# s-elkazdadi/ddp-pinocchio

Measured on AMD Instinct MI355X. Metric: DDP iterations/sec (fwd+bwd sweep), Talos nq=38 T=200, higher is better.
Workload: dtype f64

## Files before the change

ddp_pinocchio_amd/csrc/internal.h:

```cpp
#pragma once

#include <hip/hip_runtime.h>
#include <stdint.h>

#include <vector>

#include "bwd_jobs.h"
#include "cost_block.h"
#include "ddp_hip/ddp_hip.h"

#define DDP_MAXJ DDP_HIP_MAX_JOINTS

struct DevModel {
  int32_t kind, nv;
  int32_t ff, nj, nq, pad0_;
  double mass, length;
  double gravity[3];
  double dt, c;
  int32_t parent[DDP_MAXJ];
  int32_t jtype[DDP_MAXJ];
  double axis[DDP_MAXJ][3];
  double Rp[DDP_MAXJ][9];
  double pp[DDP_MAXJ][3];
  double I6[DDP_MAXJ][21];
  int32_t has_child[DDP_MAXJ];
  int32_t first_contrib[DDP_MAXJ];
  int32_t last_child[DDP_MAXJ];
  int32_t slot_up[DDP_MAXJ];
  int32_t slot_down[DDP_MAXJ];
  int32_t n_slots;
  int32_t n_levels, max_level_width;
  int32_t lvl_start[DDP_MAXJ + 1];
  int32_t lvl_joint[DDP_MAXJ];
  int32_t child_start[DDP_MAXJ + 1];
  int32_t child_list[DDP_MAXJ];
  int32_t eq_kind, eq_advance, frame_joint, first_order_fd, fd_mode, pad_;
  double frame_off[3];
};

struct Dims {
  int64_t T, n, m, nx, nv, batch;
  int64_t Etot;
  int64_t emax;
};

struct SeqBuf {
  double* ptr = nullptr;
  int64_t size = 0;
};

struct DevSwitches {
  bool generic_bwd = false;
  bool k3_no_sym = false;
  bool k3_no_half = false;
  bool k3_no_pack = false;
  bool k3h_column_jobs = false;
  bool fxx_full = false;
  bool no_static = false;
  bool no_qcache = false;
  bool qcache_dense = false;
  bool cfg_full_aba = false;
  bool ana_own_aba = false;
  bool ana_split = false;
  bool ana_eq_kernel = false;
  bool bwd_no_graph = false;
  bool solve_sync = false;
  bool fwd_no_pipe = false;
  bool lin_serial = false;
  int32_t lin_forks = 0;
  int32_t bwd_cbx = 0, bwd_cbu = 0;
  int64_t qws_bt = 0;
  int64_t ana_bt = 0;
};

struct SweepPlan {
  bool fast;
  bool sym_ok;
  bool sym;
  int32_t half_mode;
  bool packed;
};

enum class LinFirst : int32_t {
  Base,
  AnalyticSmall,
  AnalyticWave,
  AnalyticFF,
  FdStatic,
  FdGeneric,
};
enum class LinSecond : int32_t {
  None,
  Zeros,
  Mode2Static,
  Mode2Caches,
  Mode2Plain,
  Mode1Small,
  Mode1Wave,
};
enum class LinEq : int32_t {
  None,
  PerLane,
  Analytic,
  Chain,
};
enum LinFork : uint32_t {
  LIN_FORK_CFG = 1,
  LIN_FORK_SPINE = 2,
  LIN_FORK_DEFAULT = LIN_FORK_CFG | LIN_FORK_SPINE,
};
enum class LinEqJac : int32_t { None, Fd, FfLookahead };
enum class LinEqSecond : int32_t { None, Zeros, Mode2, Mode1Small, Mode1Wave };
struct LinPlan {
  int32_t refuse = 0;
  int32_t nj = 0;
  int32_t topo = 0;
  LinFirst first = LinFirst::Base;
  LinSecond second = LinSecond::None;
  LinEq eq = LinEq::None;
  LinEqJac eq_jac = LinEqJac::None;
  LinEqSecond eq_second = LinEqSecond::None;
  bool eq_inline = false;
  bool accel_static = false;
  bool accel_with_u = false;
  bool m1_fused = false;
  int32_t ncfg = 0, nvcfg = 0;
  bool qc_sparse = false;
  bool has_tensors = false;
  bool skip_top = false;
  bool skip_qv_mirror = false;
  bool pack = false;
  bool ws_lin = false, ws_qws = false, ws_qws2 = false;
  bool ws_ana_T = false, ws_ana_M = false, ws_ana_M0 = false, ws_ana_A = false, ws_ana_F = false;
  bool ws_eq = false;
  bool ana_sliced = false;
  int64_t eq_fxk_off = 0, eq_c_off = 0, eq_words = 0;
  uint32_t forks = 0;
  int32_t lin_path = 0, first_order = 0;
};
DevSwitches read_switches();
LinPlan lin_plan_decide(const DevModel& m, const Dims& d, uint32_t flags, const DevSwitches& sw, int topo_id, bool sweep_sym_ok);

enum class TensorOrigin : int32_t {
  Unknown,
  Symmetric,
  Stencil,
  Analytic1,
};
struct TensorState {
  TensorOrigin origin = TensorOrigin::Unknown;
  bool mirror_pending = false;
  bool packed = false;
};

struct LinCall {
  bool ana_A_fresh = false;
  bool ana_M0_fresh = false;
  bool fuu_zero = false;
};

struct ProfSlot {
  std::vector<hipEvent_t> starts, stops;
  size_t used = 0;
  double total_ms = 0;
  int64_t launches = 0;
};

struct ddp_hip_ctx {
  int device = 0;
  int cu_count = 0;
  uint32_t flags = 0;
  hipStream_t stream = nullptr;
  Dims d{};
  std::vector<int64_t> ne_h, Epre_h;
  int64_t* ne_d = nullptr;
  int64_t* Epre_d = nullptr;
  double* target_d = nullptr;
  DevModel model_h{};
  DevModel* model_d = nullptr;
  SeqBuf seq[DDP_HIP_SEQ_COUNT];
  DevSwitches sw;

  double* ws_V = nullptr;
  double* ws_Q = nullptr;
  double* reg_d = nullptr;
  double* mu_d = nullptr;
  int32_t* status_d = nullptr;
  int64_t* restarts_d = nullptr;
  BwdJob* jobs_d = nullptr;
  BwdJob* jobs_half_d = nullptr;
  int32_t njobs_half = 0;
  K3hUnit* units_half_d = nullptr;
  int32_t njobs_units = 0;
  TensorState tensors;
  BwdJob* jobs_sym_d = nullptr;
  int32_t njobs = 0;
  int32_t cbx = 0, cbu = 0;
  struct BwdGraph { const void* key_x = nullptr; uint64_t key_misc = 0; hipGraphExec_t exec = nullptr; hipGraph_t graph = nullptr; };
  BwdGraph bwd_graph[4];
  int bwd_graph_next = 0;

  double* fw_x = nullptr;
  double* fw_u = nullptr;
  double* fw_dcost = nullptr;
  double* fw_cost = nullptr;
  double* fw_cost_old = nullptr;
  double* step_d = nullptr;
  int32_t* fw_state_d = nullptr;
  double* fw_dcost_acc_d = nullptr;
  int32_t n_alpha_max = 8;
  double* pick_pair_d = nullptr;

  double* eq_ws = nullptr;
  double* lin_ws = nullptr;
  LinPlan plan;
  double* lin_qws = nullptr;
  int64_t lin_qws_bt = 0;
  double* lin_qws2 = nullptr;
  hipStream_t lin_stream2 = nullptr;
  hipEvent_t lin_ev_up[2] = {nullptr, nullptr}, lin_ev_dn[2] = {nullptr, nullptr};
  hipEvent_t lin_ev_fork = nullptr, lin_ev_done = nullptr, lin_ev_rows = nullptr;
  bool lin_side_busy = false;
  double* ana_T = nullptr;
  double* ana_M = nullptr;
  double* ana_F = nullptr;
  double* ana_M0 = nullptr;
  double* ana_A = nullptr;
  int64_t ana_nbt = 0;

  std::vector<int32_t> active_h;
  bool all_active = true;

  CostBlock cost[COST_COUNT];
  int32_t fc_nf = 0;
  int32_t fc_joint[DDP_HIP_MAX_COST_FRAMES] = {};
  double fc_off[DDP_HIP_MAX_COST_FRAMES][3] = {};
  int32_t ob_np = 0, ob_no = 0;
  int32_t ob_joint[DDP_HIP_MAX_COLLISION_POINTS] = {};
  double ob_off[DDP_HIP_MAX_COLLISION_POINTS][3] = {};
  double ob_radius[DDP_HIP_MAX_COLLISION_POINTS] = {};
  int32_t ob_kind[DDP_HIP_MAX_OBSTACLES] = {};
  double* ob_clear_d = nullptr;
  int32_t sc_np = 0, sc_npair = 0;
  int32_t sc_joint[DDP_HIP_MAX_COLLISION_POINTS] = {};
  double sc_off[DDP_HIP_MAX_COLLISION_POINTS][3] = {};
  double sc_radius[DDP_HIP_MAX_COLLISION_POINTS] = {};
  int32_t sc_pa[DDP_HIP_MAX_COLLISION_PAIRS] = {}, sc_pb[DDP_HIP_MAX_COLLISION_PAIRS] = {};
  double* sc_clear_d = nullptr;
  int32_t cp_nc = 0, cp_npair = 0;
  int32_t cp_joint[DDP_HIP_MAX_CAPSULES] = {};
  double cp_end[DDP_HIP_MAX_CAPSULES][2][3] = {};
  double cp_radius[DDP_HIP_MAX_CAPSULES] = {};
  int32_t cp_pa[DDP_HIP_MAX_CAPSULE_PAIRS] = {}, cp_kind[DDP_HIP_MAX_CAPSULE_PAIRS] = {}, cp_pb[DDP_HIP_MAX_CAPSULE_PAIRS] = {};
  double* cp_clear_d = nullptr;
  int32_t rf_np = 0;
  int32_t rf_ja[DDP_HIP_MAX_FRAME_PAIRS] = {}, rf_jb[DDP_HIP_MAX_FRAME_PAIRS] = {};
  double rf_offa[DDP_HIP_MAX_FRAME_PAIRS][3] = {}, rf_offb[DDP_HIP_MAX_FRAME_PAIRS][3] = {};
  double* rf_err_d = nullptr;
  int32_t fa_nf = 0;
  int32_t fa_joint[DDP_HIP_MAX_AIM_FRAMES] = {};
  double fa_off[DDP_HIP_MAX_AIM_FRAMES][3] = {}, fa_axis[DDP_HIP_MAX_AIM_FRAMES][3] = {};
  double* fa_err_d = nullptr;

  int32_t br_np = 0;
  double* ja_acc_d = nullptr;
  double* br_margin_d = nullptr;

  bool box_dirty = false;

  void* adv_tab_d = nullptr;
  double* adv_x0_d = nullptr;
  int32_t adv_narr = 0;
  int64_t adv_blocks = 0;
  bool adv_dirty = true;
  std::vector<double> adv_mu_h, adv_step_h;

  bool async_mode = false;
  uint32_t profile_mask = 0;
  ProfSlot prof[DDP_HIP_K_COUNT];
};

#define HIP_TRY(expr)                                   \
  do {                                                  \
    hipError_t e__ = (expr);                            \
    if (e__ != hipSuccess) { (void)hipGetLastError(); return DDP_HIP_E_HIP; } \
  } while (0)

#define END_SYNC(ctx) do { if (!(ctx)->async_mode) HIP_TRY(hipStreamSynchronize((ctx)->stream)); } while (0)

inline hipError_t lin_fork(ddp_hip_ctx* ctx) {
  hipError_t e = hipEventRecord(ctx->lin_ev_fork, ctx->stream);
  if (e == hipSuccess) e = hipStreamWaitEvent(ctx->lin_stream2, ctx->lin_ev_fork, 0);
  if (e == hipSuccess) ctx->lin_side_busy = true;
  return e;
}
inline hipError_t lin_join(ddp_hip_ctx* ctx) {
  if (!ctx->lin_side_busy) return hipSuccess;
  hipError_t e = hipEventRecord(ctx->lin_ev_done, ctx->lin_stream2);
  if (e == hipSuccess) e = hipStreamWaitEvent(ctx->stream, ctx->lin_ev_done, 0);
  if (e != hipSuccess) { (void)hipGetLastError(); (void)hipStreamSynchronize(ctx->lin_stream2); }
  ctx->lin_side_busy = false;
  return e;
}
struct LinJoin {
  ddp_hip_ctx* ctx;
  explicit LinJoin(ddp_hip_ctx* c) : ctx(c) {}
  LinJoin(const LinJoin&) = delete;
  LinJoin& operator=(const LinJoin&) = delete;
  ~LinJoin() { (void)lin_join(ctx); }
};

void prof_begin(ddp_hip_ctx* ctx, int kid, hipStream_t stream = nullptr);
void prof_end(ddp_hip_ctx* ctx, int kid, hipStream_t stream = nullptr);

int bwd_setup(ddp_hip_ctx* ctx);
SweepPlan sweep_plan(const ddp_hip_ctx* ctx);
void bwd_teardown(ddp_hip_ctx* ctx);
int bwd_lds_check(const ddp_hip_ctx* ctx);
int box_check(ddp_hip_ctx* ctx);
int fwd_setup(ddp_hip_ctx* ctx);
bool fwd_lat_supported(const ddp_hip_ctx* ctx);
void fwd_teardown(ddp_hip_ctx* ctx);
void adv_teardown(ddp_hip_ctx* ctx);
int lin_setup(ddp_hip_ctx* ctx);
int tensors_written_outside(ddp_hip_ctx* ctx, int seq);
int lin_materialize_fxx(ddp_hip_ctx* ctx);
void lin_teardown(ddp_hip_ctx* ctx);

int pick_local_launch(ddp_hip_ctx* ctx, int64_t rank, int64_t nranks, double* out_pair, hipStream_t stream);
int pick_final_launch(const double* pairs, int G, double* out_pair, hipStream_t stream);

static inline int64_t seq_block_offset_regular(int64_t t, int64_t stride) { return t * stride; }
```

ddp_pinocchio_amd/csrc/lin.hip:

```cpp
#include <float.h>
#include <math.h>
#include <stdlib.h>

#include "balance_region_cost.h"
#include "capsule_cost.h"
#include "com_cost.h"
#include "control_grav_cost.h"
#include "frame_aim_cost.h"
#include "frame_cost.h"
#include "frame_vel_cost.h"
#include "internal.h"
#include "joint_accel_cost.h"
#include "lin_common.h"
#include "momentum_cost.h"
#include "obstacle_cost.h"
#include "rbd.h"
#include "rbd_deriv.h"
#include "relative_frame_cost.h"
#include "self_collision_cost.h"
#include "state_limits.h"

namespace {


// ... 1101 lines not shown
    else { for (int i = m.nq; i < nx; ++i) xb[i] = xa[i]; rbd::eval_f_q<NJ>(m, xa, xb); }
    for (int i = 0; i < nx; ++i) { xa[i] = xb[i]; p.eq_xk[(gid * K + k) * nx + i] = xb[i]; }
  }
  double* C = p.eq_c + gid * (int64_t)p.d.emax * n;
  for (int i = 0; i < e * n; ++i) C[i] = 0.0;
  const double* target = p.target + Eo;
  if (m.eq_kind == DDP_HIP_EQ_CONFIG) {
    for (int i = 0; i < e; ++i) { p.eq_val[Eb + i] = xa[i] - target[i]; C[i + i * e] = 1.0; }
  } else {
    double pos[3], J[3 * NJ];
    rbd::frame_position<NJ>(m, xa, pos, J);
    for (int i = 0; i < e; ++i) p.eq_val[Eb + i] = pos[i] - target[i];
    for (int j = 0; j < nv; ++j)
      for (int i = 0; i < e; ++i) C[i + j * e] = J[i + 3 * j];
  }
}

template <int NJ>
__global__ void eq_fdjac_kernel(LinParams p) {
  const int64_t gid = (int64_t)blockIdx.x * blockDim.x + threadIdx.x;
  const int64_t T = p.d.T;
  const DevModel& m = *p.model;
  const int n = 2 * m.nv, K = m.eq_advance;
  if (K < 2 || gid >= p.d.batch * T * (K - 1) * n) return;
  const int j = (int)(gid % n);
  const int k = (int)((gid / n) % (K - 1));
  const int64_t bt = gid / ((int64_t)n * (K - 1));
  const int b = (int)(bt / T);
  const int64_t t = bt % T;
  if (p.ne[t] == 0) return;
  double x[2 * NJ + 1], u[NJ], f[2 * NJ + 1];
  const int nx = (int)p.d.nx;
  const double* xk = p.eq_xk + (bt * K + k) * nx;
  const double* xk1 = p.eq_xk + (bt * K + k + 1) * nx;
  const double* us = p.u + ((int64_t)b * T + t) * m.nv;
  for (int i = 0; i < nx; ++i) x[i] = xk[i];
  for (int i = 0; i < m.nv; ++i) u[i] = us[i];
  const double eps = sqrt(DBL_EPSILON);
  lie::perturb_x(m, x, j, eps);
  double* col = p.eq_fxk + (bt * (K - 1) + k) * (int64_t)n * n + (int64_t)j * n;
  if (k == K - 2 && !m.ff) {
    const int nv = m.nv;
    for (int i = 0; i < nv; ++i) { const double vo = m.dt * x[nv + i]; const double fq = x[i] + vo; col[i] = (fq - xk1[i]) / eps; }
    for (int i = nv; i < n; ++i) col[i] = 0.0;
    return;
  }
  rbd::eval_f<NJ>(m, x, u, f);
  if (m.ff) {
    double df[2 * NJ];
    lie::difference_x(m, xk1, f, df);
    for (int i = 0; i < n; ++i) col[i] = df[i] / eps;
  } else {
    for (int i = 0; i < n; ++i) col[i] = (f[i] - xk1[i]) / eps;
  }
}

__global__ void eq_combine_kernel(LinParams p) {
  const int64_t bt = blockIdx.x;
  const int64_t T = p.d.T;
  const int b = (int)(bt / T);
  const int64_t t = bt % T;
  const int e = (int)p.ne[t];
  if (e == 0) return;
  const int n = (int)p.d.n, mm = (int)p.d.m, K = p.model->eq_advance;
  const int64_t Eb = (int64_t)b * p.d.Etot + p.Epre[t];
  extern __shared__ double sm[];
  double* ex = sm;
  double* tmp = sm + (int64_t)p.d.emax * n;
  const double* C = p.eq_c + bt * (int64_t)p.d.emax * n;
  for (int i = threadIdx.x; i < e * n; i += blockDim.x) ex[i] = C[i];
  __syncthreads();
  for (int k = K - 2; k >= 0; --k) {
    const double* F = p.eq_fxk + (bt * (K - 1) + k) * (int64_t)n * n;
    for (int idx = threadIdx.x; idx < e * n; idx += blockDim.x) {
      const int i = idx % e, j = idx / e;
      double s = 0;
      for (int l = 0; l < n; ++l) s += ex[i + l * e] * F[l + (int64_t)j * n];
      tmp[idx] = s;
    }
    __syncthreads();
    for (int i = threadIdx.x; i < e * n; i += blockDim.x) ex[i] = tmp[i];
    __syncthreads();
  }
  const double* fx = p.fx + bt * n * n;
  const double* fu = p.fu + bt * n * mm;
  for (int idx = threadIdx.x; idx < e * n; idx += blockDim.x) {
    const int i = idx % e, j = idx / e;
    double s = 0;
    for (int l = 0; l < n; ++l) s += ex[i + l * e] * fx[l + j * n];
    p.eq_x[Eb * n + idx] = s;
  }
  for (int idx = threadIdx.x; idx < e * mm; idx += blockDim.x) {
    const int i = idx % e, j = idx / e;
    double s = 0;
    for (int l = 0; l < n; ++l) s += ex[i + l * e] * fu[l + j * n];
    p.eq_u[Eb * mm + idx] = s;
  }
}

#define MAXADV 4

template <int NJ>
__global__ void eq_first_kernel(LinParams p) {
  const int64_t gid = (int64_t)blockIdx.x * blockDim.x + threadIdx.x;
  const int64_t T = p.d.T;
  if (gid >= p.d.batch * T) return;
  const int b = (int)(gid / T);
  const int64_t t = gid % T;
  const int e = (int)p.ne[t];
  if (e == 0) return;
  const DevModel& m = *p.model;
  const int n = (int)p.d.n, mm = (int)p.d.m;
  const int64_t Eo = p.Epre[t], Eb = (int64_t)b * p.d.Etot + Eo;
  double x[2 * NJ], u[NJ];
  load_xu<NJ>(p, b, t, x, u);
  eq_first_order<NJ, MAXADV>(m, p.target + Eo, e, x, u, p.eq_x + Eb * n, p.eq_u + Eb * mm, p.eq_val + Eb);
}

template <int NJ>
__global__ void second_m1_kernel(LinParams p, int is_eq) {
  const int64_t gid = (int64_t)blockIdx.x * blockDim.x + threadIdx.x;
  const int64_t T = p.d.T;
  const int n = (int)p.d.n, mm = (int)p.d.m;
  const int W = n + mm;
  if (gid >= p.d.batch * T * W) return;
  const int i = (int)(gid % W);
  const int64_t bt = gid / W;
  const int b = (int)(bt / T);
  const int64_t t = bt % T;
  const DevModel& m = *p.model;
  constexpr int N = 2 * NJ, M = NJ, EM = NJ > 3 ? NJ : 3;
  double x[N], u[M];
  load_xu<NJ>(p, b, t, x, u);
  const double eps = sqrt(DBL_EPSILON);
  const bool at_x = i < n;
  const int idx = at_x ? i : i - n;
  if (at_x) x[idx] = x[idx] + eps; else u[idx] = u[idx] + eps;
  if (!is_eq) {
    double fx_[N * N], fu_[N * M], out_[N];
    first_order_f<NJ>(m, x, u, fx_, fu_, out_);
    const double* ox = p.fx + bt * n * n;
    const double* ou = p.fu + bt * n * mm;
    const int o = n;
    if (at_x) {
      for (int k = 0; k < o; ++k) {
        for (int j = 0; j < n; ++j) p.fxx[bt * n * n * n + k + (int64_t)j * o + (int64_t)idx * o * n] = (fx_[k + j * o] - ox[k + j * o]) / eps;
        for (int j = 0; j < mm; ++j) p.fux[bt * n * mm * n + k + (int64_t)j * o + (int64_t)idx * o * mm] = (fu_[k + j * o] - ou[k + j * o]) / eps;
      }
    } else {
      for (int k = 0; k < o; ++k)
        for (int j = 0; j < mm; ++j) p.fuu[bt * n * mm * mm + k + (int64_t)j * o + (int64_t)idx * o * mm] = (fu_[k + j * o] - ou[k + j * o]) / eps;
    }
  } else {
    const int e = (int)p.ne[t];
    if (e == 0) return;
    const int64_t Eo = p.Epre[t], Eb = (int64_t)b * p.d.Etot + Eo;
    double ex_[EM * N], eu_[EM * M], out_[EM];
    eq_first_order<NJ, MAXADV>(m, p.target + Eo, e, x, u, ex_, eu_, out_);
    const double* ox = p.eq_x + Eb * n;
    const double* ou = p.eq_u + Eb * mm;
    const int o = e;
    if (at_x) {
      for (int k = 0; k < o; ++k) {
        for (int j = 0; j < n; ++j) p.eq_xx[Eb * n * n + k + (int64_t)j * o + (int64_t)idx * o * n] = (ex_[k + j * o] - ox[k + j * o]) / eps;
        for (int j = 0; j < mm; ++j) p.eq_ux[Eb * mm * n + k + (int64_t)j * o + (int64_t)idx * o * mm] = (eu_[k + j * o] - ou[k + j * o]) / eps;
      }
    } else {
      for (int k = 0; k < o; ++k)
        for (int j = 0; j < mm; ++j) p.eq_uu[Eb * mm * mm + k + (int64_t)j * o + (int64_t)idx * o * mm] = (eu_[k + j * o] - ou[k + j * o]) / eps;
    }
  }
}

template <int NJ>
__global__ void eq_second_m2_kernel(LinParams p, int stage) {
  const int64_t gid = (int64_t)blockIdx.x * blockDim.x + threadIdx.x;
  const int64_t T = p.d.T;
  const int n = (int)p.d.n, mm = (int)p.d.m;
  const int W = n + mm;
  const int64_t P = stage == 0 ? W : (int64_t)W * (W - 1) / 2;
  if (gid >= p.d.batch * T * P) return;
  const int64_t pid = gid % P;
  const int64_t bt = gid / P;
  const int b = (int)(bt / T);
  const int64_t t = bt % T;
  const int e = (int)p.ne[t];
  if (e == 0) return;
  int i, j;
  if (stage == 0) { i = (int)pid; j = -1; }
  else {
    i = (int)floor(((2.0 * W - 1.0) - sqrt((2.0 * W - 1.0) * (2.0 * W - 1.0) - 8.0 * (double)pid)) * 0.5);
    if (i < 0) i = 0;
    while ((int64_t)i * (2 * W - i - 1) / 2 > pid) --i;
    while ((int64_t)(i + 1) * (2 * W - i - 2) / 2 <= pid) ++i;
    j = (int)(pid - (int64_t)i * (2 * W - i - 1) / 2) + i + 1;
  }
  const DevModel& m = *p.model;
  constexpr int EM = NJ > 3 ? NJ : 3;
  double x[2 * NJ + 1], u[NJ], f1[EM];
  load_xu<NJ>(p, b, t, x, u);
  const double eps = sqrt(sqrt(DBL_EPSILON));
  const double eps2 = eps * eps;
  const int64_t Eo = p.Epre[t], Eb = (int64_t)b * p.d.Etot + Eo;
  const double* f0 = p.eq_val + Eb;
  double* exx = p.eq_xx + Eb * n * n;
  double* eux = p.eq_ux + Eb * mm * n;
  double* euu = p.eq_uu + Eb * mm * mm;
  const bool at_x_1 = i < n;
  const int idx_1 = at_x_1 ? i : i - n;
  const bool both_base = stage != 0 && m.ff && i < 6 && j < 6;
  if (both_base) {
    double nu[6] = {0, 0, 0, 0, 0, 0}, q7[7];
    nu[i] = eps; nu[j] = eps;
    lie::se3_integrate(x, nu, q7);
    for (int k = 0; k < 7; ++k) x[k] = q7[k];
  } else if (at_x_1) lie::perturb_x(m, x, idx_1, eps); else u[idx_1] = u[idx_1] + eps;
  const double* fcol_1 = at_x_1 ? p.eq_x + Eb * n + (int64_t)idx_1 * e : p.eq_u + Eb * mm + (int64_t)idx_1 * e;
  const int L1 = at_x_1 ? n : mm;
  double* tensor_1 = at_x_1 ? exx : euu;
  if (stage == 0) {
    eq_eval<NJ>(m, p.target + Eo, e, x, u, f1);
    for (int k = 0; k < e; ++k) {
      double df = f1[k] - f0[k];
      df -= eps * fcol_1[k];
      df *= 2;
      tensor_1[k + (int64_t)idx_1 * e + (int64_t)idx_1 * e * L1] = df / eps2;
    }
    return;
  }
  const bool at_x_2 = j < n;
  const int idx_2 = at_x_2 ? j : j - n;
  if (both_base) {} else if (at_x_2) lie::perturb_x(m, x, idx_2, eps); else u[idx_2] = u[idx_2] + eps;
  const double* fcol_2 = at_x_2 ? p.eq_x + Eb * n + (int64_t)idx_2 * e : p.eq_u + Eb * mm + (int64_t)idx_2 * e;
  const int L2 = at_x_2 ? n : mm;
  const double* tensor_2 = at_x_2 ? exx : euu;
  double* tensor;
  int L;
  if (at_x_1) { if (at_x_2) { tensor = exx; L = n; } else { tensor = eux; L = mm; } }
  else { tensor = euu; L = mm; }
  eq_eval<NJ>(m, p.target + Eo, e, x, u, f1);
  for (int k = 0; k < e; ++k) {
    double df = f1[k] - f0[k];
    df -= eps * fcol_1[k];
    df -= eps * fcol_2[k];
    df *= 2;
    const double val = 0.5 * (df / eps2 - tensor_1[k + (int64_t)idx_1 * e + (int64_t)idx_1 * e * L1] -
                              tensor_2[k + (int64_t)idx_2 * e + (int64_t)idx_2 * e * L2]);
    tensor[k + (int64_t)idx_2 * e + (int64_t)idx_1 * e * L] = val;
    if (at_x_1 == at_x_2) tensor[k + (int64_t)idx_1 * e + (int64_t)idx_2 * e * L] = val;
  }
}

__global__ void tensor_mirror_kernel(double* Tn, int64_t BT, int n, int L) {
  const int64_t per = (int64_t)n * L * L, total = BT * per;
  for (int64_t g = (int64_t)blockIdx.x * blockDim.x + threadIdx.x; g < total; g += (int64_t)gridDim.x * blockDim.x) {
    const int64_t bt = g / per, r = g % per;
    const int k = (int)(r % n), j = (int)((r / n) % L), c = (int)(r / ((int64_t)n * L));
    if (j >= c) continue;
    double* T = Tn + bt * per;
    T[k + (int64_t)j * n + (int64_t)c * n * L] = T[k + (int64_t)c * n + (int64_t)j * n * L];
  }
}

__global__ void tensor_zero_top_kernel(double* Tn, int64_t total_cols, int n, int nv) {
  const int64_t total = total_cols * nv;
  for (int64_t g = (int64_t)blockIdx.x * blockDim.x + threadIdx.x; g < total; g += (int64_t)gridDim.x * blockDim.x) {
    const int64_t col = g / nv;
    Tn[col * n + (g % nv)] = 0.0;
  }
}

constexpr int UNPACK_BS = 256;
__global__ __launch_bounds__(UNPACK_BS) void tensor_unpack_kernel(double* fxx, double* fux, double* fuu, int n, int m, int nv) {
  extern __shared__ __attribute__((aligned(16))) double s_rec[];
  const int per = 2 * n + m;
  const int64_t bt = blockIdx.x / per;
  const int s = (int)(blockIdx.x % per);
  double* slab;
  int L, c;
  bool tops;
  if (s < n) { c = s; L = n; tops = true; slab = fxx + (bt * n + c) * (int64_t)n * n; }
  else if (s < 2 * n) { c = s - n; L = m; tops = true; slab = fux + (bt * n + c) * (int64_t)n * m; }
  else { c = s - 2 * n; L = m; tops = false; slab = fuu + (bt * m + c) * (int64_t)n * m; }
  const int R = nv + 2, words = L * R;
  for (int e = threadIdx.x; e < words; e += UNPACK_BS) s_rec[e] = slab[e];
  __syncthreads();
  const int r0 = c % nv;
  for (int e = threadIdx.x; e < L * n; e += UNPACK_BS) {
    const int j = e / n, k = e - j * n;
    const double* rec = s_rec + j * R;
    double v = 0.0;
    if (k >= nv) v = rec[2 + (k - nv)];
    else if (tops && k == r0) v = rec[0];
    else if (tops && L == n && k == j % nv) v = rec[1];
    slab[e] = v;
  }
}

int64_t lin_qc_per_bt(const ddp_hip_ctx* ctx) {
  const LinPlan& pl = ctx->plan;
  return pl.qc_sparse ? lin_static_qc_per_bt(pl.topo) : (int64_t)pl.ncfg * ctx->d.nv * rbd::QC_STRIDE;
}

LinParams make_params(ddp_hip_ctx* ctx) {
  LinParams p{};
  p.d = ctx->d;
  p.model = ctx->model_d;
  p.ne = ctx->ne_d;
  p.Epre = ctx->Epre_d;
  p.target = ctx->target_d;
  auto S = [&](int s) { return ctx->seq[s].ptr; };
  p.x = S(DDP_HIP_SEQ_X); p.u = S(DDP_HIP_SEQ_U);
  p.lfx = S(DDP_HIP_SEQ_LFX); p.lfxx = S(DDP_HIP_SEQ_LFXX);
  p.lx = S(DDP_HIP_SEQ_LX); p.lu = S(DDP_HIP_SEQ_LU); p.lxx = S(DDP_HIP_SEQ_LXX); p.lux = S(DDP_HIP_SEQ_LUX); p.luu = S(DDP_HIP_SEQ_LUU);
  p.f_val = S(DDP_HIP_SEQ_F_VAL); p.fx = S(DDP_HIP_SEQ_FX); p.fu = S(DDP_HIP_SEQ_FU);
  p.fxx = S(DDP_HIP_SEQ_FXX); p.fux = S(DDP_HIP_SEQ_FUX); p.fuu = S(DDP_HIP_SEQ_FUU);
  p.eq_val = S(DDP_HIP_SEQ_EQ_VAL); p.eq_x = S(DDP_HIP_SEQ_EQ_X); p.eq_u = S(DDP_HIP_SEQ_EQ_U);
  p.eq_xx = S(DDP_HIP_SEQ_EQ_XX); p.eq_ux = S(DDP_HIP_SEQ_EQ_UX); p.eq_uu = S(DDP_HIP_SEQ_EQ_UU);
  const LinPlan& pl = ctx->plan;
  p.has_tensors = pl.has_tensors ? 1 : 0;
  p.skip_top = pl.skip_top ? 1 : 0;
  p.skip_qv_mirror = pl.skip_qv_mirror ? 1 : 0;
  p.pack = pl.pack ? 1 : 0;
  p.eq_xk = ctx->eq_ws;
  if (p.eq_xk) { p.eq_fxk = p.eq_xk + pl.eq_fxk_off; p.eq_c = p.eq_xk + pl.eq_c_off; }
  p.qcache = ctx->lin_ws;
  p.ncfg = pl.ncfg; p.nvcfg = pl.nvcfg;
  p.qc_sparse = pl.qc_sparse ? 1 : 0;
  p.qc_bt = lin_qc_per_bt(ctx);
  p.vcache = p.qcache ? p.qcache + ctx->d.batch * ctx->d.T * p.qc_bt : nullptr;
  p.xref = S(DDP_HIP_SEQ_COST_XREF); p.wx = S(DDP_HIP_SEQ_COST_WX); p.uref = S(DDP_HIP_SEQ_COST_UREF); p.wu = S(DDP_HIP_SEQ_COST_WU);
  return p;
}

inline unsigned blocks_for(int64_t total) { return (unsigned)((total + LBS - 1) / LBS); }

template <int NJ>
int eq_second_order(ddp_hip_ctx* ctx, const LinParams& p, LinCall& call, uint32_t stages) {
  const Dims& d = ctx->d;
  const int64_t BT = d.batch * d.T;
  const int W = (int)(d.n + d.m);
  const int64_t P = (int64_t)W * (W - 1) / 2;
  switch (ctx->plan.eq_second) {
    case LinEqSecond::None: break;
    case LinEqSecond::Mode2:
      hipLaunchKernelGGL((eq_second_m2_kernel<NJ>), dim3(blocks_for(BT * W)), dim3(LBS), 0, ctx->stream, p, 0);
      hipLaunchKernelGGL((eq_second_m2_kernel<NJ>), dim3(blocks_for(BT * P)), dim3(LBS), 0, ctx->stream, p, 1);
      break;
    case LinEqSecond::Mode1Small:
      if constexpr (NJ <= 6) hipLaunchKernelGGL((second_m1_kernel<NJ>), dim3(blocks_for(BT * W)), dim3(LBS), 0, ctx->stream, p, 1);
      break;
    case LinEqSecond::Mode1Wave: {
      const int fl = LIN_ANA_EQ | ((stages & DDP_HIP_LIN_SECOND) ? LIN_ANA_F : 0);
      if (fl & LIN_ANA_F) prof_begin(ctx, DDP_HIP_K_LIN_SECOND);
      const int rc_ = lin_analytic_launch(ctx, p, call, 1, fl);
      if (fl & LIN_ANA_F) prof_end(ctx, DDP_HIP_K_LIN_SECOND);
      if (rc_ != DDP_HIP_OK) return rc_;
      break;
    }
    case LinEqSecond::Zeros:
      HIP_TRY(hipMemsetAsync(p.eq_xx, 0, sizeof(double) * (size_t)(ctx->seq[DDP_HIP_SEQ_EQ_XX].size * d.batch), ctx->stream));
      HIP_TRY(hipMemsetAsync(p.eq_ux, 0, sizeof(double) * (size_t)(ctx->seq[DDP_HIP_SEQ_EQ_UX].size * d.batch), ctx->stream));
      HIP_TRY(hipMemsetAsync(p.eq_uu, 0, sizeof(double) * (size_t)(ctx->seq[DDP_HIP_SEQ_EQ_UU].size * d.batch), ctx->stream));
      break;
  }
  return DDP_HIP_OK;
}

template <int NJ>
int run_linearize(ddp_hip_ctx* ctx, const LinParams& p, LinCall& call, uint32_t stages) {
  const LinPlan& pl = ctx->plan;
  const Dims& d = ctx->d;
  const int64_t BT = d.batch * d.T;
  const int W = (int)(d.n + d.m);
  const int nv = (int)d.nv;
  [[maybe_unused]] constexpr bool small = NJ <= 6;
  const bool second_stage = (stages & DDP_HIP_LIN_SECOND) && pl.second != LinSecond::None;
  const bool eq_stage = (stages & DDP_HIP_LIN_EQ) && pl.eq != LinEq::None;
  const bool m1_fused = pl.m1_fused && eq_stage;
  if (stages & DDP_HIP_LIN_COST) {
    if (ctx->flags & DDP_HIP_FLAG_TRACKING_COST)
      hipLaunchKernelGGL(lin_track_cost_kernel, dim3((unsigned)(BT + d.batch)), dim3(64), 0, ctx->stream, p);
    else hipLaunchKernelGGL(lin_cost_kernel, dim3((unsigned)BT), dim3(64), 0, ctx->stream, p);
    const dim3 blocks((unsigned)(BT + d.batch));
    const FrameCostDev fc = frame_cost_dev(ctx);
    const StateLimitsDev sl = state_limits_dev(ctx);
    const CoMCostDev cm = com_cost_dev(ctx);
    const FrameVelCostDev fv = frame_vel_cost_dev(ctx);
    const MomentumCostDev mo = momentum_cost_dev(ctx);
    const BalanceRegionDev br = balance_region_dev(ctx);
    const RelativeFrameDev rf = relative_frame_dev(ctx);
    const ControlGravDev cg = control_grav_dev(ctx);
    const FrameAimDev fa = frame_aim_dev(ctx);
    const JointAccelDev ja = joint_accel_dev(ctx);
    const ObstacleCostDev ob = obstacle_cost_dev(ctx);
    const SelfCollisionDev sc = self_collision_dev(ctx);
    const CapsuleCostDev cp = capsule_cost_dev(ctx);
    auto add = [&](bool live, auto kernel, const auto& dev) { if (live) hipLaunchKernelGGL(kernel, blocks, dim3(64), 0, ctx->stream, p, dev); };
    add(fc.target, lin_frame_cost_kernel, fc);
    add(fc.oquat, lin_frame_orient_cost_kernel, fc);
    add(sl.weight, lin_limit_cost_kernel, sl);
    add(cm.target, lin_com_cost_kernel, cm);
    add(fv.target, lin_frame_vel_cost_kernel, fv);
    add(mo.target, lin_momentum_cost_kernel, mo);
    add(br.geom, lin_balance_region_cost_kernel, br);
    add(rf.weight, lin_relative_frame_cost_kernel, rf);
    if (cg.weight)
      hipLaunchKernelGGL(lin_control_grav_cost_kernel, dim3((unsigned)BT), dim3(64), sizeof(double) * (size_t)(d.nv * d.nv), ctx->stream, p, cg);
    add(fa.weight, lin_frame_aim_cost_kernel, fa);
    if (ja.weight) {
      constexpr int lds = (int)(sizeof(double) * rbdd::FfLds<DDP_HIP_MAX_JOINT_ACCEL_NV>::TOTAL);
      HIP_TRY(hipFuncSetAttribute(reinterpret_cast<const void*>(&lin_joint_accel_cost_kernel<DDP_HIP_MAX_JOINT_ACCEL_NV>),
                                  hipFuncAttributeMaxDynamicSharedMemorySize, lds));
      hipLaunchKernelGGL((lin_joint_accel_cost_kernel<DDP_HIP_MAX_JOINT_ACCEL_NV>), dim3((unsigned)BT), dim3(64), lds, ctx->stream, p, ja);
    }
    add(ob.geom, lin_obstacle_cost_kernel, ob);
    add(sc.margin, lin_self_collision_cost_kernel, sc);
    add(cp.geom, lin_capsule_cost_kernel, cp);
  }
  bool caches_built = false;
  int static_rc = DDP_HIP_OK;
  auto build_caches = [&]() {
    if (caches_built) return;
    if (pl.topo) { const int rc_ = lin_static_launch(ctx, p, StaticLevel::Caches); if (rc_ != DDP_HIP_OK) static_rc = rc_; }
    else {
      hipLaunchKernelGGL((lin_qcache_kernel<NJ>), dim3(blocks_for(BT * (nv + 1))), dim3(LBS), 0, ctx->stream, p);
      hipLaunchKernelGGL((lin_vcache_kernel<NJ>), dim3(blocks_for(BT * (2 * nv + 1))), dim3(LBS), 0, ctx->stream, p);
    }
    caches_built = true;
  };
  if (stages & DDP_HIP_LIN_FIRST) {
    prof_begin(ctx, DDP_HIP_K_LIN_FIRST);
    hipLaunchKernelGGL((lin_base_kernel<NJ>), dim3(blocks_for(BT)), dim3(LBS), 0, ctx->stream, p);
    switch (pl.first) {
      case LinFirst::Base: break;
      case LinFirst::AnalyticSmall:
        if constexpr (small) hipLaunchKernelGGL((lin_first_analytic_small_kernel<NJ>), dim3(blocks_for(BT)), dim3(LBS), 0, ctx->stream, p);
        break;
      case LinFirst::AnalyticWave:
      case LinFirst::AnalyticFF: {
        const bool m1_next = pl.second == LinSecond::Mode1Wave && second_stage;
        const int rc_ = lin_analytic_launch(ctx, p, call, 0, LIN_ANA_F | (m1_next ? LIN_ANA_ACCEL : 0) | (m1_next && eq_stage ? LIN_ANA_EQ << 4 : 0));
        if (rc_ != DDP_HIP_OK) return rc_;
        break;
      }
      case LinFirst::FdStatic: {
        build_caches();
        const int rc_ = lin_static_launch(ctx, p, StaticLevel::FirstOrder);
        if (rc_ != DDP_HIP_OK) return rc_;
        break;
      }
      case LinFirst::FdGeneric:
        hipLaunchKernelGGL((lin_first_kernel<NJ>), dim3(blocks_for(BT * W)), dim3(LBS), 0, ctx->stream, p);
        break;
    }
    prof_end(ctx, DDP_HIP_K_LIN_FIRST);
  }
  if (second_stage) {
    const int64_t P = (int64_t)W * (W - 1) / 2, TRI = (int64_t)nv * (nv - 1) / 2, Pv = (int64_t)nv * nv + TRI, Pu = 2 * (int64_t)nv * nv + TRI;
    prof_begin(ctx, DDP_HIP_K_LIN_SECOND);
    switch (pl.second) {
      case LinSecond::None: break;
      case LinSecond::Mode2Static:
        build_caches();
        if (pl.forks) {
          const int rc_ = lin_static_launch(ctx, p, StaticLevel::SecondOrder);
          if (rc_ != DDP_HIP_OK) return rc_;
          break;
        }
        for (StaticLevel level : {StaticLevel::UDiagonal, StaticLevel::Torque, StaticLevel::Velocity, StaticLevel::Configuration}) {
          const int rc_ = lin_static_launch(ctx, p, level);
          if (rc_ != DDP_HIP_OK) return rc_;
        }
        break;
      case LinSecond::Mode2Caches:
        build_caches();
        hipLaunchKernelGGL((lin_diag_kernel<NJ>), dim3(blocks_for(BT * W)), dim3(LBS), 0, ctx->stream, p);
        hipLaunchKernelGGL((lin_offdiag_kernel<NJ, 3>), dim3(blocks_for(BT * Pu)), dim3(LBS), 0, ctx->stream, p);
        hipLaunchKernelGGL((lin_offdiag_kernel<NJ, 2>), dim3(blocks_for(BT * Pv)), dim3(LBS), 0, ctx->stream, p);
        hipLaunchKernelGGL((lin_offdiag_kernel<NJ, 1>), dim3(blocks_for(BT * TRI)), dim3(LBS), 0, ctx->stream, p);
        break;
      case LinSecond::Mode2Plain:
        hipLaunchKernelGGL((lin_diag_kernel<NJ>), dim3(blocks_for(BT * W)), dim3(LBS), 0, ctx->stream, p);
        hipLaunchKernelGGL((lin_offdiag_kernel<NJ, 0>), dim3(blocks_for(BT * P)), dim3(LBS), 0, ctx->stream, p);
        break;
      case LinSecond::Mode1Small:
        if constexpr (small) hipLaunchKernelGGL((second_m1_kernel<NJ>), dim3(blocks_for(BT * W)), dim3(LBS), 0, ctx->stream, p, 0);
        break;
      case LinSecond::Mode1Wave:
        if (!m1_fused) { const int rc_ = lin_analytic_launch(ctx, p, call, 1, LIN_ANA_F); if (rc_ != DDP_HIP_OK) return rc_; }
        break;
      case LinSecond::Zeros:
        HIP_TRY(hipMemsetAsync(p.fxx, 0, sizeof(double) * (size_t)(ctx->seq[DDP_HIP_SEQ_FXX].size * d.batch), ctx->stream));
        HIP_TRY(hipMemsetAsync(p.fux, 0, sizeof(double) * (size_t)(ctx->seq[DDP_HIP_SEQ_FUX].size * d.batch), ctx->stream));
        HIP_TRY(hipMemsetAsync(p.fuu, 0, sizeof(double) * (size_t)(ctx->seq[DDP_HIP_SEQ_FUU].size * d.batch), ctx->stream));
        break;
    }
    HIP_TRY(lin_join(ctx));
    prof_end(ctx, DDP_HIP_K_LIN_SECOND);
  }
  if (eq_stage) {
    switch (pl.eq) {
      case LinEq::None: break;
      case LinEq::PerLane:
        if constexpr (small) hipLaunchKernelGGL((eq_first_kernel<NJ>), dim3(blocks_for(BT)), dim3(LBS), 0, ctx->stream, p);
        break;
      case LinEq::Analytic: {
        const int rc_ = lin_analytic_launch(ctx, p, call, 0, LIN_ANA_EQ);
        if (rc_ != DDP_HIP_OK) return rc_;
        break;
      }
      case LinEq::Chain: {
        const int K = ctx->model_h.eq_advance;
        if (K < 1) return DDP_HIP_E_UNSUPPORTED;
        hipLaunchKernelGGL((eq_chain_kernel<NJ>), dim3(blocks_for(BT)), dim3(LBS), 0, ctx->stream, p);
        if (pl.eq_jac == LinEqJac::Fd) hipLaunchKernelGGL((eq_fdjac_kernel<NJ>), dim3(blocks_for(BT * (K - 1) * d.n)), dim3(LBS), 0, ctx->stream, p);
        else if (pl.eq_jac == LinEqJac::FfLookahead) { const int rc_ = lin_analytic_ff_lookahead(ctx, p); if (rc_ != DDP_HIP_OK) return rc_; }
        hipLaunchKernelGGL(eq_combine_kernel, dim3((unsigned)BT), dim3(256), sizeof(double) * (size_t)(2 * d.emax * d.n), ctx->stream, p);
        break;
      }
    }
    const int rc_ = eq_second_order<NJ>(ctx, p, call, stages);
    if (rc_ != DDP_HIP_OK) return rc_;
  }
  HIP_TRY(hipGetLastError());
  return static_rc;
}

int tensors_begin_second(ddp_hip_ctx* ctx, const LinParams& p, LinCall& call) {
  const TensorOrigin was = ctx->tensors.origin;
  ctx->tensors.origin = TensorOrigin::Unknown;
  ctx->tensors.packed = false;
  call.fuu_zero = was == TensorOrigin::Analytic1;
  if (p.skip_top && !p.pack && was != TensorOrigin::Stencil) {
    const int64_t BT = ctx->d.batch * ctx->d.T, n = ctx->d.n, m = ctx->d.m;
    const int nv = (int)ctx->d.nv;
    hipLaunchKernelGGL(tensor_zero_top_kernel, dim3(8192), dim3(256), 0, ctx->stream, p.fxx, BT * n * n, (int)n, nv);
    hipLaunchKernelGGL(tensor_zero_top_kernel, dim3(8192), dim3(256), 0, ctx->stream, p.fux, BT * m * n, (int)n, nv);
    hipLaunchKernelGGL(tensor_zero_top_kernel, dim3(8192), dim3(256), 0, ctx->stream, p.fuu, BT * m * m, (int)n, nv);
    HIP_TRY(hipGetLastError());
  }
  return DDP_HIP_OK;
}

void tensors_end_second(ddp_hip_ctx* ctx, const LinParams& p, const LinCall& call) {
  TensorState& t = ctx->tensors;
  if (ctx->model_h.fd_mode == 1) t.origin = call.fuu_zero ? TensorOrigin::Analytic1 : TensorOrigin::Unknown;
  else t.origin = p.skip_top ? TensorOrigin::Stencil : TensorOrigin::Symmetric;
  t.mirror_pending = p.skip_qv_mirror != 0;
  t.packed = p.pack != 0;
}

}

int lin_setup(ddp_hip_ctx* ctx) {
  const Dims& d = ctx->d;
  const int topo_id = ctx->model_h.kind == DDP_HIP_MODEL_TREE ? lin_static_supported(ctx->model_h) : 0;
  ctx->plan = lin_plan_decide(ctx->model_h, d, ctx->flags, ctx->sw, topo_id, sweep_plan(ctx).sym_ok);
  const LinPlan& pl = ctx->plan;
  if (pl.refuse) return pl.refuse;
  if (pl.ws_lin)
    HIP_TRY(hipMalloc(&ctx->lin_ws, sizeof(double) * (size_t)(d.batch * d.T * (lin_qc_per_bt(ctx) + (int64_t)pl.nvcfg * d.nv * rbd::VC_STRIDE))));
  if (pl.ws_qws) {
    const int64_t BT = d.batch * d.T;
    int64_t slice = (pl.forks & LIN_FORK_SPINE) ? 3200 : 1024;
    if (ctx->sw.qws_bt) slice = ctx->sw.qws_bt;
    ctx->lin_qws_bt = BT < slice ? BT : slice;
    HIP_TRY(hipMalloc(&ctx->lin_qws, sizeof(double) * (size_t)(ctx->lin_qws_bt * lin_static_ws_per_bt(ctx->model_h))));
    if (pl.ws_qws2) {
      HIP_TRY(hipMalloc(&ctx->lin_qws2, sizeof(double) * (size_t)(ctx->lin_qws_bt * lin_static_ws_per_bt(ctx->model_h))));
      HIP_TRY(hipStreamCreateWithFlags(&ctx->lin_stream2, hipStreamNonBlocking));
      for (int k = 0; k < 2; ++k) {
        HIP_TRY(hipEventCreateWithFlags(&ctx->lin_ev_up[k], hipEventDisableTiming));
        HIP_TRY(hipEventCreateWithFlags(&ctx->lin_ev_dn[k], hipEventDisableTiming));
      }
    }
  }
  if (pl.forks) {
    HIP_TRY(hipStreamCreateWithFlags(&ctx->lin_stream2, hipStreamNonBlocking));
    HIP_TRY(hipEventCreateWithFlags(&ctx->lin_ev_fork, hipEventDisableTiming));
    HIP_TRY(hipEventCreateWithFlags(&ctx->lin_ev_done, hipEventDisableTiming));
    HIP_TRY(hipEventCreateWithFlags(&ctx->lin_ev_rows, hipEventDisableTiming));
  }
  { const int rc_ = lin_analytic_setup(ctx); if (rc_ != DDP_HIP_OK) return rc_; }
  if (pl.ws_eq) HIP_TRY(hipMalloc(&ctx->eq_ws, sizeof(double) * (size_t)pl.eq_words));
  if (pl.eq == LinEq::Chain) {
    const size_t lds = sizeof(double) * (size_t)(2 * d.emax * d.n);
    if (lds > 64 * 1024) HIP_TRY(hipFuncSetAttribute(reinterpret_cast<const void*>(&eq_combine_kernel), hipFuncAttributeMaxDynamicSharedMemorySize, (int)lds));
  }
  return DDP_HIP_OK;
}
void lin_teardown(ddp_hip_ctx* ctx) {
  lin_analytic_teardown(ctx);
  for (int k = 0; k < 2; ++k) {
    if (ctx->lin_ev_up[k]) (void)hipEventDestroy(ctx->lin_ev_up[k]);
    if (ctx->lin_ev_dn[k]) (void)hipEventDestroy(ctx->lin_ev_dn[k]);
  }
  for (hipEvent_t ev : {ctx->lin_ev_fork, ctx->lin_ev_done, ctx->lin_ev_rows}) if (ev) (void)hipEventDestroy(ev);
  if (ctx->lin_stream2) (void)hipStreamDestroy(ctx->lin_stream2);
  if (ctx->lin_qws2) (void)hipFree(ctx->lin_qws2);
  if (ctx->lin_qws) (void)hipFree(ctx->lin_qws);
  if (ctx->eq_ws) (void)hipFree(ctx->eq_ws);
  if (ctx->lin_ws) (void)hipFree(ctx->lin_ws);
}

extern "C" int ddp_hip_linearize_stages(ddp_hip_ctx* ctx, uint32_t stages) {
  if (!ctx) return DDP_HIP_E_ARG;
  HIP_TRY(hipSetDevice(ctx->device));
  LinParams p = make_params(ctx);
  LinCall call;
  LinJoin joined(ctx);
  const bool second = (stages & DDP_HIP_LIN_SECOND) && p.has_tensors;
  if (second) { const int rc_ = tensors_begin_second(ctx, p, call); if (rc_ != DDP_HIP_OK) return rc_; }
  int rc;
  switch (ctx->plan.nj) {
    case 1: rc = run_linearize<1>(ctx, p, call, stages); break;
    case 6: rc = run_linearize<6>(ctx, p, call, stages); break;
    case 38: rc = run_linearize<38>(ctx, p, call, stages); break;
    default: rc = run_linearize<64>(ctx, p, call, stages); break;
  }
  if (rc != DDP_HIP_OK) return rc;
  END_SYNC(ctx);
  if (second) tensors_end_second(ctx, p, call);
  return DDP_HIP_OK;
}

int tensors_written_outside(ddp_hip_ctx* ctx, int seq) {
  if (seq != DDP_HIP_SEQ_FXX && seq != DDP_HIP_SEQ_FUX && seq != DDP_HIP_SEQ_FUU) return DDP_HIP_OK;
  TensorState& t = ctx->tensors;
  if (t.packed) { const int rc_ = lin_materialize_fxx(ctx); if (rc_ != DDP_HIP_OK) return rc_; }
  if (seq == DDP_HIP_SEQ_FUX) {
    t.origin = (t.origin == TensorOrigin::Symmetric || t.origin == TensorOrigin::Stencil) ? TensorOrigin::Symmetric : TensorOrigin::Unknown;
    return DDP_HIP_OK;
  }
  const int rc_ = lin_materialize_fxx(ctx);
  if (rc_ != DDP_HIP_OK) return rc_;
  t.origin = TensorOrigin::Unknown;
  return DDP_HIP_OK;
}

int lin_materialize_fxx(ddp_hip_ctx* ctx) {
  double* fxx = ctx->seq[DDP_HIP_SEQ_FXX].ptr;
  double* fuu = ctx->seq[DDP_HIP_SEQ_FUU].ptr;
  if (ctx->tensors.packed) {
    double* fux = ctx->seq[DDP_HIP_SEQ_FUX].ptr;
    const int64_t BT = ctx->d.batch * ctx->d.T, n = ctx->d.n, m = ctx->d.m, nv = ctx->d.nv;
    if (!fxx || !fux || !fuu || m > n) return DDP_HIP_E_UNSUPPORTED;
    hipLaunchKernelGGL(tensor_unpack_kernel, dim3((unsigned)(BT * (2 * n + m))), dim3(UNPACK_BS), sizeof(double) * (size_t)(n * (nv + 2)), ctx->stream,
                       fxx, fux, fuu, (int)n, (int)m, (int)nv);
    HIP_TRY(hipGetLastError());
    HIP_TRY(hipStreamSynchronize(ctx->stream));
    ctx->tensors.packed = false;
  }
  if (!ctx->tensors.mirror_pending) return DDP_HIP_OK;
  if (fxx && fuu) {
    const int64_t BT = ctx->d.batch * ctx->d.T;
    hipLaunchKernelGGL(tensor_mirror_kernel, dim3(8192), dim3(256), 0, ctx->stream, fxx, BT, (int)ctx->d.n, (int)ctx->d.n);
    hipLaunchKernelGGL(tensor_mirror_kernel, dim3(4096), dim3(256), 0, ctx->stream, fuu, BT, (int)ctx->d.n, (int)ctx->d.m);
    HIP_TRY(hipGetLastError());
    HIP_TRY(hipStreamSynchronize(ctx->stream));
  }
  ctx->tensors.mirror_pending = false;
  return DDP_HIP_OK;
}

extern "C" int ddp_hip_linearize(ddp_hip_ctx* ctx) {
  return ddp_hip_linearize_stages(ctx, DDP_HIP_LIN_COST | DDP_HIP_LIN_FIRST | DDP_HIP_LIN_SECOND | DDP_HIP_LIN_EQ);
}
```

ddp_pinocchio_amd/csrc/lin_common.h:

```cpp
#pragma once
#include "internal.h"

struct LinParams {
  Dims d;
  const DevModel* model;
  const int64_t* ne;
  const int64_t* Epre;
  const double* target;
  const double *x, *u;
  double *lfx, *lfxx, *lx, *lu, *lxx, *lux, *luu;
  double *f_val, *fx, *fu, *fxx, *fux, *fuu;
  double *eq_val, *eq_x, *eq_u, *eq_xx, *eq_ux, *eq_uu;
  int32_t has_tensors;
  double *eq_xk, *eq_fxk, *eq_c;
  double* vcache;
  double* qcache;
  int64_t qc_bt;
  int32_t qc_sparse;
  int32_t skip_qv_mirror;
  int32_t skip_top;
  int32_t pack;
  double* accel_out;
  int32_t ncfg, nvcfg;
  const double *xref, *wx, *uref, *wu;
};

constexpr int LBS = 64;

int lin_static_supported(const DevModel& m);
enum class StaticLevel {
  Caches,
  FirstOrder,
  UDiagonal,
  Torque,
  Velocity,
  Configuration,
  SecondOrder,
  AccelX,
  AccelXU,
};
int lin_static_launch(ddp_hip_ctx* ctx, const LinParams& p, StaticLevel level);
int64_t lin_static_ws_per_bt(const DevModel& m);
int64_t lin_static_qc_per_bt(int topo);

int lin_analytic_setup(ddp_hip_ctx* ctx);
void lin_analytic_teardown(ddp_hip_ctx* ctx);
constexpr int LIN_ANA_F = 1, LIN_ANA_EQ = 2;
constexpr int LIN_ANA_ACCEL = 4;
int lin_analytic_launch(ddp_hip_ctx* ctx, const LinParams& p, LinCall& call, int stage, int flags);
int lin_analytic_ff_lookahead(ddp_hip_ctx* ctx, const LinParams& p);
```

ddp_pinocchio_amd/csrc/lin_plan.cpp:

```cpp
#include <stdlib.h>

#include "internal.h"

DevSwitches read_switches() {
  auto on = [](const char* name) { return getenv(name) != nullptr; };
  auto knob = [](const char* name, int lo, int hi) { const char* ev = getenv(name); const int v = ev ? atoi(ev) : 0; return v >= lo && v <= hi ? v : 0; };
  DevSwitches sw;
  sw.generic_bwd = on("DDP_HIP_GENERIC_BWD");
  sw.k3_no_sym = on("DDP_HIP_K3_NO_SYM");
  sw.k3_no_half = on("DDP_HIP_K3_NO_HALF");
  sw.k3_no_pack = on("DDP_HIP_K3_NO_PACK");
  sw.k3h_column_jobs = on("DDP_HIP_K3H_COLUMN_JOBS");
  sw.fxx_full = on("DDP_HIP_FXX_FULL");
  sw.no_static = on("DDP_HIP_NO_STATIC");
  sw.no_qcache = on("DDP_HIP_NO_QCACHE");
  sw.qcache_dense = on("DDP_HIP_QCACHE_DENSE");
  sw.cfg_full_aba = on("DDP_HIP_CFG_FULL_ABA");
  sw.ana_own_aba = on("DDP_HIP_ANA_OWN_ABA");
  sw.ana_split = on("DDP_HIP_ANA_SPLIT");
  sw.ana_eq_kernel = on("DDP_HIP_ANA_EQ_KERNEL");
  sw.bwd_no_graph = on("DDP_HIP_BWD_NO_GRAPH");
  sw.solve_sync = on("DDP_HIP_SOLVE_SYNC");
  sw.fwd_no_pipe = on("DDP_HIP_FWD_NO_PIPE");
  sw.lin_serial = on("DDP_HIP_LIN_SERIAL");
  sw.lin_forks = knob("DDP_HIP_LIN_FORKS", 1, 3);
  sw.bwd_cbx = knob("DDP_HIP_BWD_CBX", 1, 8);
  sw.bwd_cbu = knob("DDP_HIP_BWD_CBU", 1, 16);
  sw.qws_bt = knob("DDP_HIP_QWS_BT", 16, 65536);
  sw.ana_bt = knob("DDP_HIP_ANA_BT", 1, 65536);
  return sw;
}

LinPlan lin_plan_decide(const DevModel& m, const Dims& d, uint32_t flags, const DevSwitches& sw, int topo_id, bool sweep_sym_ok) {
  LinPlan pl;
  const bool tree = m.kind == DDP_HIP_MODEL_TREE, ff = m.ff != 0, fo_fd = m.first_order_fd != 0;
  const bool tensors = !(flags & DDP_HIP_FLAG_NO_TENSORS);
  const bool analytic = tree && !fo_fd;
  const int mode = m.fd_mode;
  const int64_t nv = d.nv, K = m.eq_advance;
  pl.has_tensors = tensors;
  pl.nj = nv <= 1 ? 1 : (nv <= 6 && !ff) ? 6 : nv <= 38 ? 38 : 64;
  const bool small = pl.nj <= 6;
  const bool wave = analytic && !small && !ff;

  if (mode == 1 && fo_fd && tensors) pl.refuse = DDP_HIP_E_UNSUPPORTED;
  if (analytic && ff && nv > 38) pl.refuse = DDP_HIP_E_UNSUPPORTED;
  if (wave && m.max_level_width > 64) pl.refuse = DDP_HIP_E_UNSUPPORTED;
  if (wave && d.Etot > 0 && (K < 1 || K > 2)) pl.refuse = DDP_HIP_E_UNSUPPORTED;

  const int topo = (tree && !ff && !sw.no_static) ? topo_id : 0;
  const bool stencil_caches = tree && mode == 2 && tensors && !ff && !sw.no_qcache;
  const bool accel = topo && wave && mode == 1 && tensors && !sw.ana_own_aba;
  if (stencil_caches) { pl.ncfg = (int32_t)nv + 1; pl.nvcfg = 2 * (int32_t)nv + 1; }
  else if ((topo && fo_fd) || accel) { pl.ncfg = 1; pl.nvcfg = 1; }
  pl.ws_lin = pl.ncfg > 0;
  pl.topo = pl.ws_lin ? topo : 0;
  pl.ws_qws = pl.topo != 0;

  if (analytic) pl.first = small ? LinFirst::AnalyticSmall : ff ? LinFirst::AnalyticFF : LinFirst::AnalyticWave;
  else if (fo_fd) pl.first = pl.topo ? LinFirst::FdStatic : LinFirst::FdGeneric;
  else pl.first = LinFirst::Base;

  if (!tensors) pl.second = LinSecond::None;
  else if (mode == 0) pl.second = LinSecond::Zeros;
  else if (mode == 1) pl.second = small ? LinSecond::Mode1Small : LinSecond::Mode1Wave;
  else if (pl.ncfg > 1) pl.second = pl.topo ? LinSecond::Mode2Static : LinSecond::Mode2Caches;
  else pl.second = LinSecond::Mode2Plain;
  pl.ws_qws2 = pl.second == LinSecond::Mode2Static && sw.cfg_full_aba;
  pl.qc_sparse = pl.second == LinSecond::Mode2Static && !sw.qcache_dense && !sw.cfg_full_aba;
  pl.skip_top = pl.topo && mode == 2 && tensors && !sw.fxx_full;
  pl.skip_qv_mirror = pl.skip_top && sweep_sym_ok;
  pl.pack = pl.skip_qv_mirror && pl.second == LinSecond::Mode2Static && !sw.k3_no_half && !sw.k3_no_pack;

  const bool m1_wave = wave && pl.second == LinSecond::Mode1Wave;
  pl.ana_sliced = analytic && !small;
  pl.ws_ana_T = wave && sw.ana_split;
  pl.ws_ana_M = wave && (sw.ana_split || (m1_wave && d.Etot > 0));
  pl.ws_ana_M0 = m1_wave && !sw.ana_split;
  pl.ws_ana_A = pl.accel_static = accel;
  pl.accel_with_u = accel && d.Etot > 0;
  pl.ws_ana_F = m1_wave && d.Etot > 0;

  pl.ws_eq = d.Etot > 0 && tree && (fo_fd || ff);
  if (d.Etot > 0) {
    pl.eq = (small && !pl.ws_eq) ? LinEq::PerLane : wave ? LinEq::Analytic : LinEq::Chain;
    if (pl.eq == LinEq::Chain && K > 1) pl.eq_jac = fo_fd ? LinEqJac::Fd : LinEqJac::FfLookahead;
    pl.eq_second = !tensors ? LinEqSecond::None : mode == 0 ? LinEqSecond::Zeros : mode == 2 ? LinEqSecond::Mode2
                   : small ? LinEqSecond::Mode1Small : LinEqSecond::Mode1Wave;
    pl.m1_fused = m1_wave;
    pl.eq_inline = m1_wave && !sw.ana_split && m.eq_kind == DDP_HIP_EQ_CONFIG && !sw.ana_eq_kernel;
  }
  if (pl.ws_eq) {
    pl.eq_fxk_off = d.batch * d.T * K * d.nx;
    pl.eq_c_off = pl.eq_fxk_off + d.batch * d.T * (K > 1 ? K - 1 : 0) * d.n * d.n;
    pl.eq_words = pl.eq_c_off + d.batch * d.T * d.emax * d.n;
  }
  if (pl.second == LinSecond::Mode2Static && !sw.lin_serial && !sw.cfg_full_aba) pl.forks = sw.lin_forks ? (uint32_t)sw.lin_forks : (uint32_t)LIN_FORK_DEFAULT;
  pl.lin_path = tree ? 1 + pl.topo : 0;
  pl.first_order = tree ? (fo_fd ? 1 : 2) : 0;
  return pl;
}

#ifdef LIN_PLAN_TABLE
#include <stdio.h>

int main(int argc, char** argv) {
  if (argc > 1 && (argv[1][0] == 's' || argv[1][0] == 'c')) {
    DevModel m{};
    m.kind = DDP_HIP_MODEL_TREE; m.nv = 38; m.nj = 38; m.nq = 38; m.first_order_fd = 1; m.fd_mode = 2; m.max_level_width = 4;
    Dims d{};
    d.T = 3; d.batch = 2; d.nv = 38; d.n = 76; d.m = 38; d.nx = 76;
    const LinPlan p = lin_plan_decide(m, d, 0u, read_switches(), 1, true);
    if (argv[1][0] == 'c') { printf("qc_sparse %d ncfg %d nvcfg %d\n", (int)p.qc_sparse, p.ncfg, p.nvcfg); return 0; }
    printf("forks %u topo %d\n", p.forks, p.topo);
    return 0;
  }
  static const char* const sw_names[] = {"none", "generic_bwd", "k3_no_sym", "k3_no_half", "fxx_full", "no_static", "no_qcache",
                                         "cfg_full_aba", "ana_own_aba", "ana_split", "ana_eq_kernel", "bwd_no_graph", "solve_sync"};
  printf("kind nv ff fo_fd mode tensors etot eq_kind K matched sw sym_ok created refuse nj topo first second eq eq_jac eq_second "
         "eq_inline accel_static accel_with_u m1_fused ncfg nvcfg has_tensors skip_top skip_qv_mirror pack ws_lin ws_qws ws_qws2 ws_ana_T "
         "ws_ana_M ws_ana_M0 ws_ana_A ws_ana_F ws_eq ana_sliced eq_fxk_off eq_c_off eq_words lin_path first_order\n");
  printf("#");
  for (const char* s : sw_names) printf(" %s", s);
  printf("\n");
  const int nvs[] = {1, 6, 7, 38, 39, 64};
  for (int kind : {DDP_HIP_MODEL_PENDULUM, DDP_HIP_MODEL_TREE})
  for (int nv : nvs) for (int ff = 0; ff < 2; ++ff) for (int fo = 0; fo < 2; ++fo) for (int mode = 0; mode < 3; ++mode)
  for (int tensors = 0; tensors < 2; ++tensors) for (int etot = 0; etot < 2; ++etot)
  for (int eqk : {DDP_HIP_EQ_NONE, DDP_HIP_EQ_CONFIG, DDP_HIP_EQ_FRAME}) for (int K = 1; K <= 3; ++K)
  for (int matched = 0; matched < 2; ++matched) for (int s = 0; s < 13; ++s) {
    DevModel m{};
    m.kind = kind; m.nv = nv; m.ff = ff; m.nj = ff ? nv - 5 : nv; m.nq = nv + ff;
    m.first_order_fd = fo; m.fd_mode = mode; m.eq_kind = eqk; m.eq_advance = K; m.max_level_width = 4;
    Dims d{};
    d.T = 3; d.batch = 2; d.nv = nv; d.n = 2 * nv; d.m = nv; d.nx = 2 * nv + ff;
    d.emax = etot ? (eqk == DDP_HIP_EQ_CONFIG ? nv : 3) : 0; d.Etot = etot ? d.emax * d.T : 0;
    DevSwitches sw;
    bool* const sws[] = {nullptr, &sw.generic_bwd, &sw.k3_no_sym, &sw.k3_no_half, &sw.fxx_full, &sw.no_static, &sw.no_qcache,
                         &sw.cfg_full_aba, &sw.ana_own_aba, &sw.ana_split, &sw.ana_eq_kernel, &sw.bwd_no_graph, &sw.solve_sync};
    if (sws[s]) *sws[s] = true;
    const int sym_ok = nv == 38 && !sw.generic_bwd && !sw.k3_no_sym;
    const bool created = (kind == DDP_HIP_MODEL_TREE || (nv == 1 && !ff)) && (!ff || (nv >= 6 && mode != 1 && eqk != DDP_HIP_EQ_CONFIG)) &&
                         (eqk != DDP_HIP_EQ_NONE || !etot);
    const LinPlan p = lin_plan_decide(m, d, tensors ? 0u : (uint32_t)DDP_HIP_FLAG_NO_TENSORS, sw, matched && !ff ? 1 : 0, sym_ok != 0);
    printf("%d %d %d %d %d %d %d %d %d %d %d %d %d %d %d %d %d %d %d %d %d %d %d %d %d %d %d %d %d %d %d %d %d %d %d %d %d %d %d %d %d %lld %lld %lld %d %d\n",
           kind == DDP_HIP_MODEL_TREE, nv, ff, fo, mode, tensors, etot, eqk == DDP_HIP_EQ_NONE ? 0 : eqk == DDP_HIP_EQ_CONFIG ? 1 : 2, K, matched, s, sym_ok,
           (int)created, p.refuse != 0, p.nj, p.topo, (int)p.first, (int)p.second, (int)p.eq, (int)p.eq_jac, (int)p.eq_second,
           (int)p.eq_inline, (int)p.accel_static, (int)p.accel_with_u, (int)p.m1_fused, p.ncfg, p.nvcfg, (int)p.has_tensors, (int)p.skip_top,
           (int)p.skip_qv_mirror, (int)p.pack, (int)p.ws_lin, (int)p.ws_qws, (int)p.ws_qws2, (int)p.ws_ana_T, (int)p.ws_ana_M, (int)p.ws_ana_M0, (int)p.ws_ana_A,
           (int)p.ws_ana_F, (int)p.ws_eq, (int)p.ana_sliced, (long long)p.eq_fxk_off, (long long)p.eq_c_off, (long long)p.eq_words, p.lin_path, p.first_order);
  }
  return 0;
}
#endif
```

ddp_pinocchio_amd/csrc/lin_static.hip:

```cpp
#include <float.h>
#include <math.h>
#include <stdlib.h>

#include <type_traits>
#include <utility>

#include "internal.h"
#include "lin_common.h"
#include "rbd.h"

#ifndef DEV_NO_EMIT
#define DEV_NO_EMIT 0
#endif
namespace {

struct TopoTalos38 {
  static constexpr int N = 38;
  static constexpr int parent[N] = {-1, 0, 1, 2, 3, 4,
                                    5, 6, 7, 8, 9, 10,
                                    5, 12, 13, 14, 15, 16,
                                    5, 18,
                                    19, 20, 21, 22, 23, 24, 25, 26,
                                    19, 28, 29, 30, 31, 32, 33, 34,
                                    19, 36};
  static constexpr int prismatic[N] = {1, 1, 1, 0, 0, 0, 0, 0, 0, 0, 0, 0, 0, 0, 0, 0, 0, 0, 0,
                                       0, 0, 0, 0, 0, 0, 0, 0, 0, 0, 0, 0, 0, 0, 0, 0, 0, 0, 0};
};

struct TopoChain6 {
  static constexpr int N = 6;
  static constexpr int parent[N] = {-1, 0, 1, 2, 3, 4};
  static constexpr int prismatic[N] = {0, 0, 0, 0, 0, 0};
};

}
#include "topo_extra.h"
namespace {

template <class T> constexpr bool has_child(int k) {
  for (int c = k + 1; c < T::N; ++c) if (T::parent[c] == k) return true;
  return false;
}
template <class T> constexpr int largest_child(int k) {
  int r = -1;
  for (int c = k + 1; c < T::N; ++c) if (T::parent[c] == k) r = c;
  return r;
}
template <class T> constexpr bool first_contrib(int k) { return T::parent[k] >= 0 && largest_child<T>(T::parent[k]) == k; }

template <class T>
bool topo_matches(const DevModel& m) {
  if (m.kind != DDP_HIP_MODEL_TREE || m.nv != T::N) return false;
  for (int i = 0; i < T::N; ++i)
    if (m.parent[i] != T::parent[i] || (m.jtype[i] == DDP_HIP_JOINT_PRISMATIC) != (T::prismatic[i] != 0)) return false;
  return true;
}

template <class T>
struct QcLayout {
  static constexpr int N = T::N, ER = 12, UD = rbd::QC_STRIDE - ER;
  static constexpr int max_depth() {
    int best = 1;
    for (int k = 0; k < N; ++k) { int d = 0; for (int a = T::parent[k]; a >= 0; a = T::parent[a]) ++d; if (d > best) best = d; }
    return best;
  }
  static constexpr int MAXD = max_depth();
  static constexpr int DW = ER + MAXD * UD;
  static constexpr int DELTA = N * rbd::QC_STRIDE, WORDS = DELTA + N * DW;
  static constexpr int PATH0 = DELTA + ER;
};
template <class T> struct AncTab { unsigned long long anc[T::N]; };
template <class T> constexpr AncTab<T> make_anc_tab() {
  static_assert(T::N <= 64, "ancestor masks are 64 bits wide");
  AncTab<T> t{};
  for (int k = 0; k < T::N; ++k) for (int a = T::parent[k]; a >= 0; a = T::parent[a]) t.anc[k] |= 1ull << a;
  return t;
}
template <class T> __device__ const AncTab<T> g_anc_tab = make_anc_tab<T>();
template <class T>
__device__ __forceinline__ int qc_word(int g, unsigned long long anc, int K, int e) {
  using L = QcLayout<T>;
  const int d = __popcll(anc & ((1ull << K) - 1ull));
  const int base = K * rbd::QC_STRIDE + e, own = L::DELTA + g * L::DW + e, path = L::PATH0 + g * L::DW + d * L::UD + (e - L::ER);
  const int w_own = (int)(e < L::ER) & (int)(K == g), w_path = (int)(e >= L::ER) & (int)((anc >> K) & 1ull);
  return base + w_own * (own - base) + w_path * (path - base);
}
template <class T>
struct TauState {
  double acc[T::N][6];
  double uu[T::N];
};

template <class T, int K, int QS>
__device__ __forceinline__ void tau_up(const DevModel& m, const double* __restrict__ qc, const double* __restrict__ vc,
                                       double tauK, TauState<T>& s) {
  constexpr int o = T::prismatic[K] ? 3 : 0;
  const double* E = qc + K * QS;
  const double* r = E + 9;
  const double* U = E + 12;
  const double dinv = E[18];
  const double* pA0 = vc + K * rbd::VC_STRIDE + 6;
  const double* Iac = vc + K * rbd::VC_STRIDE + 12;
  const double* a = m.axis[K];
  double pAi[6];
  if constexpr (has_child<T>(K)) {
#pragma unroll
    for (int k = 0; k < 6; ++k) pAi[k] = s.acc[K][k];
  } else {
#pragma unroll
    for (int k = 0; k < 6; ++k) pAi[k] = pA0[k];
  }
  double sp = 0;
#pragma unroll
  for (int k = 0; k < 3; ++k) sp += a[k] * pAi[o + k];
  const double ui = tauK - sp;
  s.uu[K] = ui;
  constexpr int par = T::parent[K];
  if constexpr (par >= 0) {
    double pa[6], fp[6];
#pragma unroll
    for (int k = 0; k < 6; ++k) pa[k] = pAi[k] + Iac[k] + U[k] * (ui * dinv);
    rbd::xform_force_T(E, r, pa, fp);
    if constexpr (first_contrib<T>(K)) {
      const double* pp0 = vc + par * rbd::VC_STRIDE + 6;
#pragma unroll
      for (int k = 0; k < 6; ++k) s.acc[par][k] = pp0[k] + fp[k];
    } else {
#pragma unroll
      for (int k = 0; k < 6; ++k) s.acc[par][k] += fp[k];
    }
  }
  if constexpr (QS == rbd::QC_STRIDE || (K % 2) == 0) __builtin_amdgcn_sched_barrier(0);
}

template <class T, int K, int QS>
__device__ __forceinline__ void tau_down(const DevModel& m, const double* __restrict__ qc, const double* __restrict__ vc,
                                         TauState<T>& s) {
  constexpr int o = T::prismatic[K] ? 3 : 0;
  const double* E = qc + K * QS;
  const double* r = E + 9;
  const double* U = E + 12;
  const double dinv = E[18];
  const double* cb = vc + K * rbd::VC_STRIDE;
  double ap[6];
  constexpr int par = T::parent[K];
  if constexpr (par >= 0) rbd::xform_motion(E, r, s.acc[par], ap);
  else {
    const double a0[6] = {0, 0, 0, -m.gravity[0], -m.gravity[1], -m.gravity[2]};
    rbd::xform_motion(E, r, a0, ap);
  }
  double sum = 0;
#pragma unroll
  for (int k = 0; k < 6; ++k) { ap[k] += cb[k]; sum += U[k] * ap[k]; }
  const double qd = (s.uu[K] - sum) * dinv;
  s.uu[K] = qd;
  if constexpr (has_child<T>(K)) {
    const double* a = m.axis[K];
#pragma unroll
    for (int k = 0; k < 6; ++k) s.acc[K][k] = ap[k];
    s.acc[K][o] += a[0] * qd; s.acc[K][o + 1] += a[1] * qd; s.acc[K][o + 2] += a[2] * qd;
  }
  if constexpr (QS == rbd::QC_STRIDE || (K % 2) == 0) __builtin_amdgcn_sched_barrier(0);
}

template <class T, int QS, class TauFn, int... Ks>
__device__ __forceinline__ void tau_up_all(const DevModel& m, const double* __restrict__ qc, const double* __restrict__ vc, TauFn tau,
                                           TauState<T>& s, std::integer_sequence<int, Ks...>) {
  (tau_up<T, T::N - 1 - Ks, QS>(m, qc, vc, tau(T::N - 1 - Ks), s), ...);
}
template <class T, int QS, int HI, class TauFn, int... Ks>
__device__ __forceinline__ void tau_up_range(const DevModel& m, const double* __restrict__ qc, const double* __restrict__ vc, TauFn tau,
                                             TauState<T>& s, std::integer_sequence<int, Ks...>) {
  (tau_up<T, HI - Ks, QS>(m, qc, vc, tau(HI - Ks), s), ...);
}
template <class T, int QS, int... Ks>
__device__ __forceinline__ void tau_down_all(const DevModel& m, const double* __restrict__ qc, const double* __restrict__ vc,
                                             TauState<T>& s, std::integer_sequence<int, Ks...>) {
  (tau_down<T, Ks, QS>(m, qc, vc, s), ...);
}

constexpr int PS = 20;
template <int NV>
__device__ __forceinline__ void stage_placements(double* sp, const double* __restrict__ qc, int lane) {
  for (int idx = lane; idx < NV * 19; idx += LBS) {
    const int K = idx / 19, e = idx - K * 19;
    sp[K * PS + e] = qc[K * rbd::QC_STRIDE + e];
  }
}

template <class T> constexpr bool parents_at_least(int from, int lo) {
  for (int k = from; k < T::N; ++k) if (T::parent[k] < lo) return false;
  return true;
}
template <class T> constexpr int stage_split() {
  for (int kh = T::N / 2; kh > 0; --kh) if (parents_at_least<T>(kh + 1, kh)) return kh;
  return 0;
}

template <int NV, int K0, int K1, bool WITH_V = true>
struct StageRegs {
  static constexpr int NPW = (K1 - K0) * 19, NVW = WITH_V ? (K1 - K0) * rbd::VC_STRIDE : 0;
  static constexpr int CP = (NPW + LBS - 1) / LBS, CV = (NVW + LBS - 1) / LBS;
  double rp[CP], rv[CV > 0 ? CV : 1];
  __device__ __forceinline__ void load(const double* __restrict__ qc, const double* __restrict__ vc, int lane) {
#pragma unroll
    for (int c = 0; c < CP; ++c) {
      int idx = c * LBS + lane;
      idx = idx < NPW ? idx : NPW - 1;
      const int K = K0 + idx / 19, e = idx % 19;
      rp[c] = qc[K * rbd::QC_STRIDE + e];
    }
#pragma unroll
    for (int c = 0; c < CV; ++c) {
      int idx = c * LBS + lane;
      idx = idx < NVW ? idx : NVW - 1;
      rv[c] = vc[K0 * rbd::VC_STRIDE + idx];
    }
  }
  template <class T>
  __device__ __forceinline__ void load_sparse(const double* __restrict__ qc0, int g, unsigned long long anc, const double* __restrict__ vc, int lane) {
#pragma unroll
    for (int c = 0; c < CP; ++c) {
      int idx = c * LBS + lane;
      idx = idx < NPW ? idx : NPW - 1;
      const int K = K0 + idx / 19, e = idx % 19;
      rp[c] = qc0[qc_word<T>(g, anc, K, e)];
    }
#pragma unroll
    for (int c = 0; c < CV; ++c) {
      int idx = c * LBS + lane;
      idx = idx < NVW ? idx : NVW - 1;
      rv[c] = vc[K0 * rbd::VC_STRIDE + idx];
    }
  }
  __device__ __forceinline__ void park(double* sp, double* sv, int lane) const {
#pragma unroll
    for (int c = 0; c < CP; ++c) {
      int idx = c * LBS + lane;
      idx = idx < NPW ? idx : NPW - 1;
      const int K = K0 + idx / 19, e = idx % 19;
      sp[K * PS + e] = rp[c];
    }
#pragma unroll
    for (int c = 0; c < CV; ++c) {
      int idx = c * LBS + lane;
      idx = idx < NVW ? idx : NVW - 1;
      sv[K0 * rbd::VC_STRIDE + idx] = rv[c];
    }
  }
};

__device__ __forceinline__ void tri_index(int64_t q, int Wd, int& ii, int& jj) {
  int a = (int)floor(((2.0 * Wd - 1.0) - sqrt((2.0 * Wd - 1.0) * (2.0 * Wd - 1.0) - 8.0 * (double)q)) * 0.5);
  if (a < 0) a = 0;
  while ((int64_t)a * (2 * Wd - a - 1) / 2 > q) --a;
  while ((int64_t)(a + 1) * (2 * Wd - a - 2) / 2 <= q) ++a;
  ii = a;
  jj = (int)(q - (int64_t)a * (2 * Wd - a - 1) / 2) + a + 1;
}

template <int NV> __device__ __forceinline__ int rec_row(bool pack, int k, int r0) { return !pack ? k : (k >= NV ? k - NV + 2 : (k == r0 ? 0 : 1)); }
template <int NV> __device__ __forceinline__ bool rec_zero(bool pack, int k, int r0) { return pack && k < NV && k != r0; }

template <int NV, int NP = LBS>
struct OutStage {
  double qdd[NP * (NV + 1)];
  int pij[NP];
};

template <int NV, int NP, bool PACK, bool UU>
__device__ __forceinline__ void offdiag_emit_as(const LinParams& p, OutStage<NV, NP>& S, bool valid, int i, int j, int64_t bt,
                                                const double* __restrict__ xg, double dt, int pass) {
  constexpr int n = 2 * NV, mm = NV;
  constexpr int RW = 16, NJ = (n + RW - 1) / RW, GRP = LBS / RW, PPG = NP / GRP, NB = NP == LBS ? 2 : 1;
  static_assert(PPG % NB == 0, "points per group");
  const double eps = sqrt(sqrt(DBL_EPSILON));
  const double eps2 = eps * eps;
  const int lane = threadIdx.x;
  if (lane / NP == pass) S.pij[lane % NP] = i | (j << 8) | ((valid ? 1 : 0) << 16);
  double* const fxx = p.fxx + bt * n * n * n;
  double* const fux = p.fux + bt * n * mm * n;
  double* const fuu = p.fuu + bt * n * mm * mm;
  const double* const fxb = p.fx + bt * n * n;
  const double* const fub = p.fu + bt * n * mm;
  __syncthreads();
  const int kk = lane % RW, grp = lane / RW;
  const double* f0 = p.f_val + bt * n;
  constexpr bool pack = PACK, uu = UU && PACK;
  const bool skip_top = PACK || p.skip_top != 0;
  constexpr int cs = pack ? NV + 2 : n;
  double f0k[NJ], xk[NJ], xvk[NJ];
#pragma unroll
  for (int jx = 0; jx < NJ; ++jx) {
    const int k = kk + RW * jx;
    const int kc = k < n ? k : n - 1;
    f0k[jx] = f0[kc];
    xk[jx] = xg[kc];
    xvk[jx] = kc < NV ? xg[NV + kc] : 0.0;
  }
  if (DEV_NO_EMIT) return;
  for (int pt = 0; pt < PPG; pt += NB) {
    double a1[NB][NJ], a2[NB][NJ], d1[NB][NJ], d2[NB][NJ];
    double* o0[NB];
    double* o1[NB];
    int ie[NB], je[NB], ee[NB], r2[NB];
#pragma unroll
    for (int u = 0; u < NB; ++u) {
      const int e = (pt + u) * GRP + grp;
      ee[u] = e;
      const int pk = S.pij[e];
      const int i1 = pk & 255, j1 = (pk >> 8) & 255;
      ie[u] = i1;
      je[u] = j1;
      const bool at_x_1 = !uu && i1 < n, at_x_2 = !uu && j1 < n;
      const int idx_1 = at_x_1 ? i1 : i1 - n, idx_2 = at_x_2 ? j1 : j1 - n;
      double* tensor;
      int L;
      if (at_x_1) { if (at_x_2) { tensor = fxx; L = n; } else { tensor = fux; L = mm; } }
      else { tensor = fuu; L = mm; }
      r2[u] = at_x_1 ? idx_1 % NV : -1;
      o0[u] = (pk >> 16) ? tensor + (int64_t)idx_2 * cs + (int64_t)idx_1 * n * L : nullptr;
      o1[u] = ((pk >> 16) && at_x_1 == at_x_2 && !p.skip_qv_mirror) ? tensor + (int64_t)idx_1 * n + (int64_t)idx_2 * n * L : nullptr;
      if (o0[u]) {
        const double* q0 = at_x_1 ? fxb + (int64_t)idx_1 * n : fub + (int64_t)idx_1 * n;
        const double* q1 = at_x_2 ? fxb + (int64_t)idx_2 * n : fub + (int64_t)idx_2 * n;
        const double* q2 = at_x_1 ? fxx + (int64_t)idx_1 * cs + (int64_t)idx_1 * n * n : fuu + (int64_t)idx_1 * cs + (int64_t)idx_1 * n * mm;
        const double* q3 = at_x_2 ? fxx + (int64_t)idx_2 * cs + (int64_t)idx_2 * n * n : fuu + (int64_t)idx_2 * cs + (int64_t)idx_2 * n * mm;
        const int r3 = at_x_2 ? idx_2 % NV : -1;
#pragma unroll
        for (int jx = 0; jx < NJ; ++jx) {
          const int k = kk + RW * jx;
          const int kc = k < n ? k : n - 1;
          a1[u][jx] = q0[kc]; a2[u][jx] = q1[kc];
          const double v2 = q2[rec_row<NV>(pack, kc, r2[u])], v3 = q3[rec_row<NV>(pack, kc, r3)];
          d1[u][jx] = rec_zero<NV>(pack, kc, r2[u]) ? 0.0 : v2;
          d2[u][jx] = rec_zero<NV>(pack, kc, r3) ? 0.0 : v3;
        }
      }
    }
#pragma unroll
    for (int u = 0; u < NB; ++u) {
      if (!o0[u]) continue;
#pragma unroll
      for (int jx = 0; jx < NJ; ++jx) {
        const int k = kk + RW * jx;
        if (k >= n) continue;
        if (skip_top && k < NV && (uu || !((ie[u] < n && ie[u] % NV == k) || (je[u] < n && je[u] % NV == k)))) continue;
        double xs = k == ie[u] ? xk[jx] + eps : xk[jx];
        if (k == je[u]) xs = xs + eps;
        double fv;
        if (k < NV) {
          double xv = (NV + k) == ie[u] ? xvk[jx] + eps : xvk[jx];
          if (NV + k == je[u]) xv = xv + eps;
          const double vo = dt * xv;
          fv = xs + vo;
        } else {
          fv = xs + S.qdd[ee[u] * (NV + 1) + (k - NV)] * dt;
        }
        double df = fv - f0k[jx];
        df -= eps * a1[u][jx];
        df -= eps * a2[u][jx];
        df *= 2;
        const double val = 0.5 * (df / eps2 - d1[u][jx] - d2[u][jx]);
        o0[u][rec_row<NV>(pack, k, r2[u])] = val;
        if (o1[u]) o1[u][k] = val;
      }
    }
  }
}

template <int NV, int NP>
__device__ __forceinline__ void offdiag_emit(const LinParams& p, OutStage<NV, NP>& S, bool valid, int i, int j, int64_t bt,
                                             const double* __restrict__ xg, double dt, int pass = 0) {
  if (p.pack) offdiag_emit_as<NV, NP, true, false>(p, S, valid, i, j, bt, xg, dt, pass);
  else offdiag_emit_as<NV, NP, false, false>(p, S, valid, i, j, bt, xg, dt, pass);
}

template <int NV>
struct RowStage {
  double q[(NV + 2) * (NV + 1)];
};

template <int NV, bool DIAG_ROW, class ST>
__device__ __forceinline__ void rowblock_emit(const ST& S, int lane, int i, int jb, double* __restrict__ out, double* __restrict__ mirror,
                                              int64_t mstride, const double* __restrict__ a2, const double* __restrict__ d2, int64_t dstride,
                                              double dt, const double* __restrict__ f0g, const double* __restrict__ a1g,
                                              double* __restrict__ d1g, const double* __restrict__ xg, bool skip_top = false, bool pack = false) {
  constexpr int n = 2 * NV, RW = 16, NJ = (n + RW - 1) / RW, CG = LBS / RW, NIT = (NV + CG - 1) / CG;
  const int r1 = i % NV;
  const int cs = pack ? NV + 2 : n;
  const double eps = sqrt(sqrt(DBL_EPSILON));
  const double eps2 = eps * eps;
  const int kk = lane % RW, cg = lane / RW;
  double xk[NJ], xvk[NJ], f0k[NJ], a1k[NJ], d1k[NJ];
#pragma unroll
  for (int j = 0; j < NJ; ++j) {
    const int k = kk + RW * j;
    const int kc = k < n ? k : n - 1;
    f0k[j] = f0g[kc];
    a1k[j] = a1g[kc];
    double x = xg[kc];
    if (kc == i) x = x + eps;
    xk[j] = x;
    double xv = xg[kc < NV ? NV + kc : kc];
    if (NV + kc == i) xv = xv + eps;
    xvk[j] = xv;
    if constexpr (DIAG_ROW) {
      double fv;
      if (kc < NV) {
        const double vo = dt * xv;
        fv = x + vo;
      } else {
        fv = x + S.q[NV * (NV + 1) + (kc - NV)] * dt;
      }
      double df = fv - f0k[j];
      df -= eps * a1k[j];
      df *= 2;
      const double dd = df / eps2;
      d1k[j] = dd;
      if (cg == 0 && k < n && !(skip_top && k < NV && k != r1)) d1g[rec_row<NV>(pack, k, r1)] = dd;
    } else {
      const double v = d1g[rec_row<NV>(pack, kc, r1)];
      d1k[j] = rec_zero<NV>(pack, kc, r1) ? 0.0 : v;
    }
  }
  double va2[2][NJ], vd2[2][NJ];
  auto fetch = [&](int it, double (&A)[NJ], double (&D)[NJ]) {
    const int c = it * CG + cg;
    const int cc = c < NV ? c : NV - 1;
    const int rd = jb + cc < n ? (jb + cc) % NV : -1;
#pragma unroll
    for (int j = 0; j < NJ; ++j) {
      const int k = kk + RW * j;
      const int kc = k < n ? k : n - 1;
      A[j] = a2[kc + cc * n];
      const double v = d2[rec_row<NV>(pack, kc, rd) + cc * dstride];
      D[j] = rec_zero<NV>(pack, kc, rd) ? 0.0 : v;
    }
  };
  auto form = [&](int it, const double (&A)[NJ], const double (&D)[NJ]) {
    const int c = it * CG + cg;
    const bool cv = c < NV;
    const int cc = cv ? c : NV - 1;
    const int jp = jb + cc;
#pragma unroll
    for (int j = 0; j < NJ; ++j) {
      const int k = kk + RW * j;
      if (!(cv && k < n)) continue;
      if (skip_top && k < NV && k != r1 && !(jp < n && jp % NV == k)) continue;
      double x = xk[j];
      if (k == jp) x = x + eps;
      double fv;
      if (k < NV) {
        double xv = xvk[j];
        if (NV + k == jp) xv = xv + eps;
        const double vo = dt * xv;
        fv = x + vo;
      } else {
        fv = x + S.q[cc * (NV + 1) + (k - NV)] * dt;
      }
      double df = fv - f0k[j];
      df -= eps * a1k[j];
      df -= eps * A[j];
      df *= 2;
      const double val = 0.5 * (df / eps2 - d1k[j] - D[j]);
      out[rec_row<NV>(pack, k, r1) + c * cs] = val;
      if (mirror) mirror[k + c * mstride] = val;
    }
  };
  if (DEV_NO_EMIT) return;
  fetch(0, va2[0], vd2[0]);
  for (int it = 0; it < NIT; it += 2) {
    if (it + 1 < NIT) fetch(it + 1, va2[1], vd2[1]);
    form(it, va2[0], vd2[0]);
    if (it + 1 < NIT) {
      if (it + 2 < NIT) fetch(it + 2, va2[0], vd2[0]);
      form(it + 1, va2[1], vd2[1]);
    }
  }
}

typedef __attribute__((address_space(4))) const LinParams* kernarg_t;
__device__ __forceinline__ kernarg_t kernarg_params() { return (kernarg_t)__builtin_amdgcn_kernarg_segment_ptr(); }
__device__ __forceinline__ LinParams emit_params() {
  const kernarg_t kp = kernarg_params();
  LinParams po;
  po.f_val = kp->f_val; po.fx = kp->fx; po.fu = kp->fu; po.fxx = kp->fxx; po.fux = kp->fux; po.fuu = kp->fuu; po.skip_qv_mirror = kp->skip_qv_mirror; po.skip_top = kp->skip_top; po.pack = kp->pack;
  return po;
}

template <class T, bool ROWS, bool PACK = false, bool SP = false>
__global__ __launch_bounds__(LBS, ROWS ? 1 : 3) void lin_static_tau_kernel(LinParams p) {
  constexpr int nv = T::N, n = 2 * nv;
  constexpr int TRI = nv * (nv - 1) / 2, GU = (TRI + LBS - 1) / LBS, G = ROWS ? 2 * nv : GU;
  const int64_t bt = blockIdx.x / G;
  const int g = (int)(blockIdx.x % G) + (ROWS ? 0 : 2 * nv);
  const int lane = threadIdx.x;
  const int64_t Tn = p.d.T;
  const int b = (int)(bt / Tn);
  const int64_t t = bt % Tn;
  const DevModel& m = *p.model;
  int i, j, cfg, vcfg;
  bool valid;
  if (g < nv) { i = g; j = n + lane; cfg = 1 + g; vcfg = nv + 1 + g; valid = lane < nv; }
  else if (g < 2 * nv) { i = g; j = n + lane; cfg = 0; vcfg = 1 + (g - nv); valid = lane < nv; }
  else {
    const int pid = (g - 2 * nv) * LBS + lane;
    valid = pid < TRI;
    tri_index(valid ? pid : 0, nv, i, j);
    i += n; j += n; cfg = 0; vcfg = 0;
  }
  const double eps = sqrt(sqrt(DBL_EPSILON));
  static_assert(ROWS || !SP, "the pairs read the base block alone");
  const double* __restrict__ qc = p.qcache + bt * p.qc_bt + (SP ? 0 : cfg * (nv * rbd::QC_STRIDE));
  const double* __restrict__ vc = p.vcache + (bt * (2 * nv + 1) + vcfg) * (int64_t)nv * rbd::VC_STRIDE;
  const double* __restrict__ xg = p.x + ((int64_t)b * (Tn + 1) + t) * n;
  const double* __restrict__ ug = p.u + ((int64_t)b * Tn + t) * nv;
  const int iu = i - n, ju = j - n;
  const int gq = cfg - 1;
  [[maybe_unused]] const unsigned long long ganc = SP && cfg > 0 ? g_anc_tab<T>.anc[gq] : 0ull;
  __shared__ union TauLds { double P[nv * PS + nv * rbd::VC_STRIDE]; RowStage<nv> S; OutStage<nv, LBS / 2> O; } s_lds;
  double* s_P = s_lds.P;
  double* s_V = s_P + nv * PS;
  constexpr int KH = stage_split<T>();
  StageRegs<nv, 0, (KH > 0) ? KH : 1> lower;
  {
    StageRegs<nv, KH, nv> upper;
    if constexpr (SP) { upper.template load_sparse<T>(qc, gq, ganc, vc, lane); lower.template load_sparse<T>(qc, gq, ganc, vc, lane); }
    else { upper.load(qc, vc, lane); lower.load(qc, vc, lane); }
    upper.park(s_P, s_V, lane);
    rbd::coop_sync<true>();
  }
  TauState<T> s;
  auto tau = [&](int k) { double v = ug[k]; if (k == iu) v = v + eps; if (k == ju) v = v + eps; return v; };
  static_assert(parents_at_least<T>(KH + 1, KH), "the first half of the pass must not reach below record KH");
  tau_up_range<T, PS, nv - 1>(m, s_P, s_V, tau, s, std::make_integer_sequence<int, nv - 1 - KH>{});
  lower.park(s_P, s_V, lane);
  rbd::coop_sync<true>();
  tau_up_range<T, PS, KH>(m, s_P, s_V, tau, s, std::make_integer_sequence<int, KH + 1>{});
  tau_down_all<T, PS>(m, s_P, s_V, s, std::make_integer_sequence<int, nv>{});
  __builtin_amdgcn_sched_barrier(0);
  if constexpr (ROWS) {
    const kernarg_t kp = kernarg_params();
    RowStage<nv>& S = s_lds.S;
    const int mm = nv;
    __syncthreads();
    const int row = lane <= nv ? lane : nv + 1;
#pragma unroll
    for (int k = 0; k < nv; ++k) S.q[row * (nv + 1) + k] = s.uu[k];
    __syncthreads();
    const bool pack = kp->pack != 0;
    const int64_t cs = pack ? nv + 2 : n;
    rowblock_emit<nv, true>(S, lane, i, n, kp->fux + bt * n * mm * n + (int64_t)i * n * mm, nullptr, 0, kp->fu + bt * n * mm,
                            kp->fuu + bt * n * mm * mm, cs + (int64_t)n * mm, m.dt, kp->f_val + bt * n,
                            kp->fx + bt * n * n + (int64_t)i * n, kp->fxx + bt * n * n * n + (int64_t)i * cs + (int64_t)i * n * n, xg, kp->skip_top != 0, pack);
  } else {
    OutStage<nv, LBS / 2>& S = s_lds.O;
    const LinParams po = emit_params();
    const double dt = m.dt;
    __syncthreads();
#pragma unroll 1
    for (int pass = 0; pass < 2; ++pass) {
      if (pass) __syncthreads();
      if (lane / (LBS / 2) == pass) {
#pragma unroll
        for (int k = 0; k < nv; ++k) S.qdd[(lane % (LBS / 2)) * (nv + 1) + k] = s.uu[k];
      }
      offdiag_emit_as<nv, LBS / 2, PACK, true>(po, S, valid, i, j, bt, xg, dt, pass);
    }
  }
}

template <class T> constexpr int n_children(int k) {
  int c = 0;
  for (int j = k + 1; j < T::N; ++j) if (T::parent[j] == k) ++c;
  return c;
}
template <class T> constexpr bool chain_start(int k) { return T::parent[k] < 0 || T::parent[k] != k - 1 || n_children<T>(T::parent[k]) > 1; }
template <class T> constexpr bool chain_end(int k) { return k == T::N - 1 || chain_start<T>(k + 1); }
template <class T> constexpr int chain_first(int k) { while (!chain_start<T>(k)) --k; return k; }
template <class T> constexpr int max_chain() {
  int best = 1;
  for (int k = 0; k < T::N; ++k)
    if (chain_end<T>(k)) { const int len = k - chain_first<T>(k) + 1; if (len > best) best = len; }
  return best;
}


template <int o>
__device__ __forceinline__ void step_joint_motion(const double* a, double vK, double* vJ) {
#pragma unroll
  for (int k = 0; k < 6; ++k) vJ[k] = 0.0;
  vJ[o] = a[0] * vK; vJ[o + 1] = a[1] * vK; vJ[o + 2] = a[2] * vK;
}
template <bool ROOT>
__device__ __forceinline__ void step_link_vel(const double* E, const double* r, const double* vel_par, const double* vJ, double* vel) {
  if constexpr (!ROOT) rbd::xform_motion(E, r, vel_par, vel);
  else {
#pragma unroll
    for (int k = 0; k < 6; ++k) vel[k] = 0.0;
  }
#pragma unroll
  for (int k = 0; k < 6; ++k) vel[k] += vJ[k];
}
__device__ __forceinline__ void step_bias_force0(const double* I6, const double* vel, double* pA) {
  double Iv[6];
  rbd::sym6_mv(I6, vel, Iv);
  rbd::crf(vel, Iv, pA);
}
template <int o>
__device__ __forceinline__ void step_U_dinv(const double* IA, const double* a, double* U, double& dinv) {
  double d = 0;
#pragma unroll
  for (int r = 0; r < 6; ++r) U[r] = IA[rbd::sidx(r, o)] * a[0] + IA[rbd::sidx(r, o + 1)] * a[1] + IA[rbd::sidx(r, o + 2)] * a[2];
#pragma unroll
  for (int k = 0; k < 3; ++k) d += a[k] * U[o + k];
  dinv = 1.0 / d;
}
__device__ __forceinline__ void step_Ia(const double* IA, const double* U, double dinv, double* Ia) {
#pragma unroll
  for (int r = 0; r < 6; ++r)
#pragma unroll
    for (int cc = 0; cc <= r; ++cc) Ia[rbd::sidx(r, cc)] = IA[rbd::sidx(r, cc)] - U[r] * U[cc] * dinv;
}
template <int o>
__device__ __forceinline__ double step_u(const double* a, const double* pA, const double* tauK) {
  double sp = 0;
#pragma unroll
  for (int k = 0; k < 3; ++k) sp += a[k] * pA[o + k];
  return *tauK - sp;
}
__device__ __forceinline__ void step_force_up(const double* E, const double* r, const double* pA, const double* Iac, const double* U,
                                              double ui, double dinv, double* fp) {
  double pa[6];
#pragma unroll
  for (int k = 0; k < 6; ++k) pa[k] = pA[k] + Iac[k] + U[k] * (ui * dinv);
  rbd::xform_force_T(E, r, pa, fp);
}
template <class T, int K>
__device__ __forceinline__ void step_accel(const DevModel* m, const double* E, const double* r, const double* U, double dinv, double vK,
                                           double& uK, double (&vel_all)[T::N][6], double (&acc_all)[T::N][6]) {
  constexpr int o = T::prismatic[K] ? 3 : 0;
  constexpr int par = T::parent[K];
  const double* a = m->axis[K];
  double vJ[6], vel[6], cb[6], ap[6];
  step_joint_motion<o>(a, vK, vJ);
  if constexpr (par >= 0) {
    rbd::xform_motion(E, r, vel_all[par], vel);
    rbd::xform_motion(E, r, acc_all[par], ap);
  } else {
    const double a0[6] = {0, 0, 0, -m->gravity[0], -m->gravity[1], -m->gravity[2]};
#pragma unroll
    for (int k = 0; k < 6; ++k) vel[k] = 0.0;
    rbd::xform_motion(E, r, a0, ap);
  }
#pragma unroll
  for (int k = 0; k < 6; ++k) vel[k] += vJ[k];
  rbd::crm(vel, vJ, cb);
  double sum = 0;
#pragma unroll
  for (int k = 0; k < 6; ++k) { ap[k] += cb[k]; sum += U[k] * ap[k]; }
  const double qd = (uK - sum) * dinv;
  uK = qd;
  if constexpr (has_child<T>(K)) {
#pragma unroll
    for (int k = 0; k < 6; ++k) { vel_all[K][k] = vel[k]; acc_all[K][k] = ap[k]; }
    acc_all[K][o] += a[0] * qd; acc_all[K][o + 1] += a[1] * qd; acc_all[K][o + 2] += a[2] * qd;
  }
}
__device__ __forceinline__ void step_vpart(const double* I6, const double* Ia, const double* vel, const double* vJ, double* rec) {
  rbd::crm(vel, vJ, rec);
  step_bias_force0(I6, vel, rec + 6);
  rbd::sym6_mv(Ia, rec, rec + 12);
}

template <class T>
struct VelState {
  double vel[T::N][6];
  double acc[T::N][6];
  double uu[T::N];
};

template <int UQS_, int QS_ = rbd::QC_STRIDE>
struct VelCtx {
  static constexpr int UQS = UQS_;
  static constexpr int QS = QS_;
  static constexpr bool V_STEPPED = true;
  static constexpr bool LDS_VEL = false;
  const DevModel* m;
  const double* qp;
  const double* __restrict__ qc;
  const double* __restrict__ xg;
  const double* __restrict__ ug;
  double* uq;
  int i, j;
  double eps;
  template <int K> __device__ __forceinline__ const double* er(double*) const { return qp + K * QS; }
  template <int K> __device__ __forceinline__ const double* er_down(double* b) const { return er<K>(b); }
  template <int K> __device__ __forceinline__ const double* ud() const { return qp + K * QS + 12; }
  template <int K> __device__ __forceinline__ void ia_cb(const double*, const double* cb, double* Iac) const { rbd::sym6_mv(qc + K * rbd::QC_STRIDE + 19, cb, Iac); }
  template <int K> __device__ __forceinline__ const double* ud_down() const { return ud<K>(); }
};

template <int NV, class C>
__device__ __forceinline__ double lane_v(const C& c, int K) {
  double v = c.xg[NV + K];
  if constexpr (C::V_STEPPED) {
    if (NV + K == c.i) v = v + c.eps;
    if (NV + K == c.j) v = v + c.eps;
  }
  return v;
}

template <class T, int K, class C>
__device__ __forceinline__ void joint_vel(const C& c, const double* E, const double* vel_par, double* vel) {
  double vJ[6];
  step_joint_motion<T::prismatic[K] ? 3 : 0>(c.m->axis[K], lane_v<T::N>(c, K), vJ);
  step_link_vel<(T::parent[K] < 0)>(E, E + 9, vel_par, vJ, vel);
}
template <class T, int K, class C>
__device__ __forceinline__ void vel_from_root(const C& c, double* vel) {
  double Pb[12], vp[6];
  if constexpr (T::parent[K] >= 0) vel_from_root<T, T::parent[K]>(c, vp);
  const double* E = c.template er<K>(Pb);
  joint_vel<T, K>(c, E, vp, vel);
}

template <class T, int K, int E, class C>
__device__ __forceinline__ void chain_down(const C& c, VelState<T>& s) {
  double Pb[12];
  joint_vel<T, K>(c, c.template er<K>(Pb), s.vel[T::parent[K] >= 0 ? T::parent[K] : 0], s.vel[K]);
  __builtin_amdgcn_sched_barrier(0);
  if constexpr (K < E) chain_down<T, K + 1, E>(c, s);
}
template <class T, int K, int F, int E, class C>
__device__ __forceinline__ void chain_down_lds(const C& c, double* cur) {
  double Pb[12], vel[6];
  joint_vel<T, K>(c, c.template er<K>(Pb), cur, vel);
#pragma unroll
  for (int k = 0; k < 6; ++k) { cur[k] = vel[k]; c.lvel[((K - F) * 6 + k) * LBS] = vel[k]; }
  __builtin_amdgcn_sched_barrier(0);
  if constexpr (K < E) chain_down_lds<T, K + 1, F, E>(c, cur);
}
template <class T, int K, int F, class C>
__device__ __forceinline__ void chain_vel_load(const C& c, const double (&vel_all)[T::N][6], double* vel) {
  if constexpr (K >= F) {
#pragma unroll
    for (int k = 0; k < 6; ++k) vel[k] = c.lvel[((K - F) * 6 + k) * LBS];
  } else {
#pragma unroll
    for (int k = 0; k < 6; ++k) vel[k] = vel_all[K][k];
  }
}

template <class T, int K, int F, class C>
__device__ __forceinline__ void chain_up(const C& c, VelState<T>& s) {
  constexpr int o = T::prismatic[K] ? 3 : 0;
  double Pb[12];
  const double* E = c.template er<K>(Pb);
  const double* r = E + 9;
  const double* U = c.template ud<K>();
  const double dinv = U[6];
  const double* a = c.m->axis[K];
  double pAi[6];
  if constexpr (has_child<T>(K)) {
#pragma unroll
    for (int k = 0; k < 6; ++k) pAi[k] = s.acc[K][k];
  } else {
    step_bias_force0(c.m->I6[K], s.vel[K], pAi);
  }
  const double ui = step_u<o>(a, pAi, c.ug + K);
  if constexpr (C::UQS == 0) s.uu[K] = ui; else c.uq[K * C::UQS] = ui;
  constexpr int par = T::parent[K];
  if constexpr (par >= 0) {
    double vJ[6], cb[6], Iac[6], fp[6];
    step_joint_motion<o>(a, lane_v<T::N>(c, K), vJ);
    rbd::crm(s.vel[K], vJ, cb);
    c.template ia_cb<K>(U, cb, Iac);
    step_force_up(E, r, pAi, Iac, U, ui, dinv, fp);
    if constexpr (first_contrib<T>(K)) {
      double p0[6];
      step_bias_force0(c.m->I6[par], s.vel[par], p0);
#pragma unroll
      for (int k = 0; k < 6; ++k) s.acc[par][k] = p0[k] + fp[k];
    } else {
#pragma unroll
      for (int k = 0; k < 6; ++k) s.acc[par][k] += fp[k];
    }
  }
  __builtin_amdgcn_sched_barrier(0);
  if constexpr (K > F) chain_up<T, K - 1, F>(c, s);
}

template <class T, int K, class C, class S>
__device__ __forceinline__ void chain_at(const C& c, S& s) {
  if constexpr (chain_end<T>(K)) {
    constexpr int F = chain_first<T>(K), P = T::parent[F];
    if constexpr (P >= 0) {
      if constexpr (first_contrib<T>(F) && n_children<T>(P) > 1) vel_from_root<T, P>(c, s.vel[P]);
    }
    if constexpr (C::LDS_VEL) {
      double cur[6] = {0, 0, 0, 0, 0, 0};
      if constexpr (P >= 0) {
#pragma unroll
        for (int k = 0; k < 6; ++k) cur[k] = s.vel[P][k];
      }
      chain_down_lds<T, F, F, K>(c, cur);
    } else {
      chain_down<T, F, K>(c, s);
    }
    chain_up<T, K, F>(c, s);
  }
}
template <class T, class C, class S, int... Ks>
__device__ __forceinline__ void chains_up_all(const C& c, S& s, std::integer_sequence<int, Ks...>) {
  (chain_at<T, T::N - 1 - Ks>(c, s), ...);
}

template <class T, int K, class C>
__device__ __forceinline__ void vel_down(const C& c, VelState<T>& s) {
  double Pb[12];
  const double* E = c.template er_down<K>(Pb);
  const double* U = c.template ud_down<K>();
  double* uK;
  if constexpr (C::UQS == 0) uK = &s.uu[K]; else uK = c.uq + K * C::UQS;
  step_accel<T, K>(c.m, E, E + 9, U, U[6], lane_v<T::N>(c, K), *uK, s.vel, s.acc);
  __builtin_amdgcn_sched_barrier(0);
}
template <class T, class C, int... Ks>
__device__ __forceinline__ void vel_down_all(const C& c, VelState<T>& s, std::integer_sequence<int, Ks...>) {
  (vel_down<T, Ks>(c, s), ...);
// ... 12 lines not shown
  const int lane = threadIdx.x;
  const int64_t Tn = p.d.T;
  const int b = (int)(bt / Tn);
  const int64_t t = bt % Tn;
  int i, j, cfg;
  bool valid;
  if (ROWS) { i = g; j = nv + lane; cfg = 1 + g; valid = lane < nv; }
  else {
    const int pid = g * LBS + lane;
    valid = pid < TRI;
    tri_index(valid ? pid : 0, nv, i, j);
    i += nv; j += nv; cfg = 0;
  }
  struct PairStage { OutStage<nv, LBS / 2> O; double spare[nv + 1]; };
  using Stage = typename std::conditional<ROWS, RowStage<nv>, PairStage>::type;
  __shared__ union VelLds { Stage S; double P[nv * rbd::QC_STRIDE]; } s_lds;
  Stage& S = s_lds.S;
  double* s_P = s_lds.P;
  VelCtx<0, rbd::QC_STRIDE> c;
  c.m = p.model;
  c.qc = p.qcache + bt * p.qc_bt + (SP ? 0 : cfg * (nv * rbd::QC_STRIDE));
  c.qp = s_P;
  c.xg = p.x + ((int64_t)b * (Tn + 1) + t) * n;
  c.ug = p.u + ((int64_t)b * Tn + t) * nv;
  c.i = i; c.j = j;
  c.eps = sqrt(sqrt(DBL_EPSILON));
  c.uq = nullptr;
  {
    constexpr int NW = nv * rbd::QC_STRIDE, CW = (NW + LBS - 1) / LBS;
    double rq[CW];
    [[maybe_unused]] const unsigned long long ganc = SP ? g_anc_tab<T>.anc[g] : 0ull;
#pragma unroll
    for (int r = 0; r < CW; ++r) {
      int idx = r * LBS + lane;
      idx = idx < NW ? idx : NW - 1;
      if constexpr (SP) idx = qc_word<T>(g, ganc, idx / rbd::QC_STRIDE, idx % rbd::QC_STRIDE);
      rq[r] = c.qc[idx];
    }
#pragma unroll
    for (int r = 0; r < CW; ++r) { const int idx = r * LBS + lane; s_P[idx < NW ? idx : NW - 1] = rq[r]; }
    c.qc = s_P;
    rbd::coop_sync<true>();
  }
  VelState<T> s;
  chains_up_all<T>(c, s, std::make_integer_sequence<int, nv>{});
  vel_down_all<T>(c, s, std::make_integer_sequence<int, nv>{});
  __builtin_amdgcn_sched_barrier(0);
  const double dt = c.m->dt;
  if constexpr (ROWS) {
    const kernarg_t kp = kernarg_params();
    double* fxx = kp->fxx + bt * n * n * n;
    const double* fxb = kp->fx + bt * n * n;
    __syncthreads();
    const int row = valid ? lane : nv;
#pragma unroll
    for (int k = 0; k < nv; ++k) S.q[row * (nv + 1) + k] = s.uu[k];
    __syncthreads();
    const bool pack = kp->pack != 0;
    const int64_t cs = pack ? nv + 2 : n;
    rowblock_emit<nv, false>(S, lane, i, nv, fxx + (int64_t)nv * cs + (int64_t)i * n * n,
                             kp->skip_qv_mirror ? nullptr : fxx + (int64_t)i * n + (int64_t)nv * n * n, (int64_t)n * n,
                             fxb + (int64_t)nv * n, fxx + (int64_t)nv * cs + (int64_t)nv * n * n, cs + (int64_t)n * n, dt,
                             kp->f_val + bt * n, fxb + (int64_t)i * n, fxx + (int64_t)i * cs + (int64_t)i * n * n, c.xg, kp->skip_top != 0, pack);
  } else {
    constexpr int NP = LBS / 2;
    const LinParams po = emit_params();
    __syncthreads();
    double* const own = &S.O.qdd[(lane % NP) * (nv + 1)];
    double* const row = lane < NP ? own : S.spare;
#pragma unroll
    for (int k = 0; k < nv; ++k) row[k] = s.uu[k];
#pragma unroll 1
    for (int pass = 0; pass < 2; ++pass) {
      if (pass) {
        __syncthreads();
        if (lane >= NP) {
#pragma unroll
          for (int k = 0; k < nv; ++k) own[k] = s.uu[k];
        }
      }
      offdiag_emit<nv, NP>(po, S.O, valid, i, j, bt, c.xg, dt, pass);
    }
  }
}

constexpr int WS_PER_JOINT = 8;

template <class T>
struct CfgState {
  double vel[T::N][6];
  double accP[T::N][6];
  double accI[T::N][21];
  double w[2][WS_PER_JOINT];
};

template <class T>
struct CfgCtx {
  static constexpr bool V_STEPPED = false;
  static constexpr bool LDS_VEL = true;
  const DevModel* __restrict__ m;
  const double* __restrict__ qc0;
  const double* __restrict__ xg;
  const double* __restrict__ ug;
  double* __restrict__ W;
  double* lvel;
  int i, j;
  const double* own;
  template <int K> __device__ __forceinline__ const double* er(double* P) const {
    const double* base = qc0 + K * rbd::QC_STRIDE;
    const double* pert = own ? own : qc0 + ((int64_t)(1 + K) * T::N + K) * rbd::QC_STRIDE;
    const bool mine = K == i || K == j;
#pragma unroll
    for (int e = 0; e < 12; ++e) P[e] = mine ? pert[e] : base[e];
    return P;
  }
};

template <class T, int K, int F>
__device__ __forceinline__ void chain_up(const CfgCtx<T>& c, CfgState<T>& s) {
  constexpr int o = T::prismatic[K] ? 3 : 0;
  const double* a = c.m->axis[K];
  double IA[21], pAi[6], U[6], velK[6], dinv;
  chain_vel_load<T, K, F>(c, s.vel, velK);
  if constexpr (has_child<T>(K)) {
#pragma unroll
    for (int k = 0; k < 21; ++k) IA[k] = s.accI[K][k];
#pragma unroll
    for (int k = 0; k < 6; ++k) pAi[k] = s.accP[K][k];
  } else {
#pragma unroll
    for (int k = 0; k < 21; ++k) IA[k] = c.m->I6[K][k];
    step_bias_force0(c.m->I6[K], velK, pAi);
  }
  step_U_dinv<o>(IA, a, U, dinv);
  const double ui = step_u<o>(a, pAi, c.ug + K);
#pragma unroll
  for (int k = 0; k < 6; ++k) c.W[(K * WS_PER_JOINT + k) * LBS] = U[k];
  c.W[(K * WS_PER_JOINT + 6) * LBS] = dinv;
  c.W[(K * WS_PER_JOINT + 7) * LBS] = ui;
  constexpr int par = T::parent[K];
  if constexpr (par >= 0) {
    double Pb[12], Ia[21], vJ[6], cb[6], Iac[6], fp[6];
    const double* P = c.template er<K>(Pb);
    step_joint_motion<o>(a, lane_v<T::N>(c, K), vJ);
    step_Ia(IA, U, dinv, Ia);
    rbd::crm(velK, vJ, cb);
    rbd::sym6_mv(Ia, cb, Iac);
    step_force_up(P, P + 9, pAi, Iac, U, ui, dinv, fp);
    if constexpr (first_contrib<T>(K)) {
      double velP[6];
      chain_vel_load<T, par, F>(c, s.vel, velP);
#pragma unroll
      for (int k = 0; k < 21; ++k) s.accI[par][k] = c.m->I6[par][k];
      step_bias_force0(c.m->I6[par], velP, s.accP[par]);
    }
    rbd::add_xtix(P, P + 9, Ia, s.accI[par]);
#pragma unroll
    for (int k = 0; k < 6; ++k) s.accP[par][k] += fp[k];
  }
  __builtin_amdgcn_sched_barrier(0);
  if constexpr (K > F) chain_up<T, K - 1, F>(c, s);
}

template <int STRIDE_>
struct CfgDownOut { double* uq; static constexpr int STRIDE = STRIDE_; };

template <class T, int K, class O>
__device__ __forceinline__ void cfg_down(const CfgCtx<T>& c, CfgState<T>& s, const O& out) {
  if constexpr (K + 1 < T::N) {
#pragma unroll
    for (int e = 0; e < WS_PER_JOINT; ++e) s.w[(K + 1) & 1][e] = c.W[((K + 1) * WS_PER_JOINT + e) * LBS];
  }
  const double* U = s.w[K & 1];
  const double vK = lane_v<T::N>(c, K);
  double Pb[12], uK = U[7];
  const double* P = c.template er<K>(Pb);
  step_accel<T, K>(c.m, P, P + 9, U, U[6], vK, uK, s.vel, s.accP);
  out.uq[K * (O::STRIDE == LBS ? LBS : 1)] = uK;
  __builtin_amdgcn_sched_barrier(0);
}
template <class T, class O, int... Ks>
__device__ __forceinline__ void cfg_down_all(const CfgCtx<T>& c, CfgState<T>& s, const O& out, std::integer_sequence<int, Ks...>) {
  (cfg_down<T, Ks>(c, s, out), ...);
}

template <class T>
__device__ __forceinline__ void cfg_setup(CfgCtx<T>& c, const LinParams& p, const DevModel* __restrict__ model, const double* __restrict__ qcache,
                                          const double* __restrict__ xs, const double* __restrict__ us, double* __restrict__ ws,
                                          int64_t bt0, int64_t& bt, bool& valid) {
  constexpr int nv = T::N, n = 2 * nv;
  constexpr int TRI = nv * (nv - 1) / 2, GU = (TRI + LBS - 1) / LBS;
  bt = bt0 + blockIdx.x / GU;
  const int g = (int)(blockIdx.x % GU);
  const int lane = threadIdx.x;
  const int64_t Tn = p.d.T;
  const int b = (int)(bt / Tn);
  const int64_t t = bt % Tn;
  const int pid = g * LBS + lane;
  valid = pid < TRI;
  tri_index(valid ? pid : 0, nv, c.i, c.j);
  c.m = model;
  c.qc0 = qcache + bt * p.qc_bt;
  c.xg = xs + ((int64_t)b * (Tn + 1) + t) * n;
  c.ug = us + ((int64_t)b * Tn + t) * nv;
  c.W = ws + (int64_t)blockIdx.x * (nv * WS_PER_JOINT * LBS) + lane;
  c.own = nullptr;
}

template <class T>
__global__ __launch_bounds__(LBS) void lin_static_cfg_up_kernel(LinParams p, const DevModel* __restrict__ model, const double* __restrict__ qcache,
                                                                const double* __restrict__ xs, const double* __restrict__ us,
                                                                double* __restrict__ ws, int64_t bt0) {
  constexpr int nv = T::N;
  constexpr int MAXCH = max_chain<T>();
  __shared__ double s_vel[MAXCH * 6 * LBS];
  CfgCtx<T> c;
  int64_t bt;
  bool valid;
  cfg_setup<T>(c, p, model, qcache, xs, us, ws, bt0, bt, valid);
  c.lvel = s_vel + threadIdx.x;
  CfgState<T> s;
  chains_up_all<T>(c, s, std::make_integer_sequence<int, nv>{});
}

template <class T>
__global__ __launch_bounds__(LBS) void lin_static_cfg_down_kernel(LinParams p, const DevModel* __restrict__ model, const double* __restrict__ qcache,
                                                                  const double* __restrict__ xs, const double* __restrict__ us,
                                                                  double* __restrict__ ws, int64_t bt0) {
  constexpr int nv = T::N;
  __shared__ OutStage<nv> S;
  CfgCtx<T> c;
  int64_t bt;
  bool valid;
  cfg_setup<T>(c, p, model, qcache, xs, us, ws, bt0, bt, valid);
  c.lvel = nullptr;
  CfgState<T> s;
#pragma unroll
  for (int e = 0; e < WS_PER_JOINT; ++e) s.w[0][e] = c.W[e * LBS];
  CfgDownOut<nv + 1> o{&S.qdd[threadIdx.x * (nv + 1)]};
  cfg_down_all<T>(c, s, o, std::make_integer_sequence<int, nv>{});
  __builtin_amdgcn_sched_barrier(0);
  offdiag_emit<nv, LBS>(emit_params(), S, valid, c.i, c.j, bt, c.xg, model->dt);
}

constexpr int SREC = 13;

template <class T>
struct SpineTab {
  static constexpr int N = T::N, TRI = N * (N - 1) / 2;
  static_assert(N >= 2 && N <= 64, "ancestor masks are 64 bits wide");
  unsigned long long mask[N];
  unsigned long long anc[N];
  int depth[N];
  int nrec;
  short pi[TRI], pj[TRI];
  short top[TRI];
  int rbase[TRI], rstride[TRI];
};
template <class T>
constexpr SpineTab<T> make_spine_tab() {
  SpineTab<T> t{};
  for (int k = 0; k < T::N; ++k)
    for (int a = T::parent[k]; a >= 0; a = T::parent[a]) { ++t.depth[k]; t.mask[a] |= 1ull << k; t.anc[k] |= 1ull << a; }
  int cnt[T::N + 2] = {}, start[T::N + 2] = {}, goff[T::N + 2] = {};
  for (int i = 0; i < T::N; ++i)
    for (int j = i + 1; j < T::N; ++j) {
      int a = T::parent[i];
      while (a >= 0 && !((t.mask[a] >> j) & 1)) a = T::parent[a];
      ++cnt[a + 1];
    }
  for (int g = 0; g <= T::N; ++g) {
    start[g + 1] = start[g] + cnt[g];
    goff[g + 1] = goff[g] + cnt[g] * (g == 0 ? 0 : t.depth[g - 1] + 1);
  }
  t.nrec = goff[T::N + 1];
  int fill[T::N + 2] = {};
  for (int i = 0; i < T::N; ++i)
    for (int j = i + 1; j < T::N; ++j) {
      int a = T::parent[i];
      while (a >= 0 && !((t.mask[a] >> j) & 1)) a = T::parent[a];
      const int g = a + 1, rank = fill[g]++, slot = start[g] + rank;
      t.pi[slot] = (short)i; t.pj[slot] = (short)j; t.top[slot] = (short)a;
      t.rbase[slot] = goff[g] + rank;
      t.rstride[slot] = cnt[g];
    }
  return t;
}
template <class T> __device__ const SpineTab<T> g_spine_tab = make_spine_tab<T>();
template <class T> constexpr unsigned long long desc_mask(int k) { return make_spine_tab<T>().mask[k]; }
template <class T> constexpr int depth_of(int k) { return make_spine_tab<T>().depth[k]; }
template <class T> constexpr int spine_records() { return make_spine_tab<T>().nrec; }
template <class T> constexpr bool spine_joint(int k) { const unsigned long long mk = desc_mask<T>(k); return (mk & (mk - 1)) != 0; }

template <int GU>
__device__ __forceinline__ bool xcd_slot(int nb, int& btl, int& g) {
  const int x = (int)blockIdx.x, s = x >> 3;
  btl = (s / GU) * 8 + (x & 7);
  g = s % GU;
  return btl < nb;
}

template <class T, bool SP>
__global__ __launch_bounds__(LBS) void lin_static_spine_kernel(const DevModel* __restrict__ model, const double* __restrict__ qcache, int64_t qc_bt,
                                                               const double* __restrict__ vcache, double* __restrict__ spine, int64_t bt0, int nb) {
  constexpr int nv = T::N, TRI = nv * (nv - 1) / 2, GU = (TRI + LBS - 1) / LBS, NREC = spine_records<T>();
  int btl, g;
  if (!xcd_slot<GU>(nb, btl, g)) return;
  const int slot = g * LBS + (int)threadIdx.x;
  if (slot >= TRI) return;
  const SpineTab<T>& tab = g_spine_tab<T>;
  const DevModel& m = *model;
  const int i = tab.pi[slot], j = tab.pj[slot];
  const int rstride = tab.rstride[slot];
  [[maybe_unused]] const unsigned long long anc_i = tab.anc[i], anc_j = tab.anc[j];
  const double* __restrict__ qc0 = qcache + (bt0 + btl) * qc_bt;
  const double* __restrict__ vc0 = vcache + ((bt0 + btl) * (2 * nv + 1)) * (int64_t)nv * rbd::VC_STRIDE;
  double* __restrict__ out = spine + ((int64_t)btl * NREC + tab.rbase[slot]) * SREC;
  double Ia[21];
#pragma unroll
  for (int k = 0; k < 21; ++k) Ia[k] = 0.0;
  int prev = -1;
  for (int K = tab.top[slot]; K >= 0; K = m.parent[K]) {
    double IA[21];
#pragma unroll
    for (int k = 0; k < 21; ++k) IA[k] = m.I6[K][k];
    for (int sl = m.child_start[K]; sl < m.child_start[K + 1]; ++sl) {
      const int c = m.child_list[sl];
      const unsigned long long mc = tab.mask[c];
      const int cfg_p = (c == i || c == j) ? 1 + c : 0;
      const int cfg_i = ((mc >> i) & 1) ? 1 + i : (((mc >> j) & 1) ? 1 + j : 0);
      const double *Pg, *Ig;
      if constexpr (SP) {
        using L = QcLayout<T>;
        Pg = qc0 + (cfg_p ? L::DELTA + c * L::DW : c * rbd::QC_STRIDE);
        const int dc = __popcll((((mc >> i) & 1) ? anc_i : anc_j) & ((1ull << c) - 1ull));
        Ig = qc0 + (cfg_i ? L::PATH0 + (cfg_i - 1) * L::DW + dc * L::UD + 7 : c * rbd::QC_STRIDE + 19);
      } else {
        Pg = qc0 + ((int64_t)cfg_p * nv + c) * rbd::QC_STRIDE;
        Ig = qc0 + ((int64_t)cfg_i * nv + c) * rbd::QC_STRIDE + 19;
      }
      double P[12], Ic[21];
#pragma unroll
      for (int k = 0; k < 12; ++k) P[k] = Pg[k];
#pragma unroll
      for (int k = 0; k < 21; ++k) { const double v = Ig[k]; Ic[k] = c == prev ? Ia[k] : v; }
      rbd::add_xtix(P, P + 9, Ic, IA);
    }
    const bool pris = m.jtype[K] == DDP_HIP_JOINT_PRISMATIC;
    const double* a = m.axis[K];
    double U[6], d = 0;
#pragma unroll
    for (int r = 0; r < 6; ++r) {
      const double u0 = IA[rbd::sidx(r, 0)] * a[0] + IA[rbd::sidx(r, 1)] * a[1] + IA[rbd::sidx(r, 2)] * a[2];
      const double u3 = IA[rbd::sidx(r, 3)] * a[0] + IA[rbd::sidx(r, 4)] * a[1] + IA[rbd::sidx(r, 5)] * a[2];
      U[r] = pris ? u3 : u0;
    }
#pragma unroll
    for (int k = 0; k < 3; ++k) d += a[k] * (pris ? U[3 + k] : U[k]);
    const double dinv = 1.0 / d;
#pragma unroll
    for (int r = 0; r < 6; ++r)
#pragma unroll
      for (int cc = 0; cc <= r; ++cc) Ia[rbd::sidx(r, cc)] = IA[rbd::sidx(r, cc)] - U[r] * U[cc] * dinv;
    double cb[6], Iac[6];
#pragma unroll
    for (int k = 0; k < 6; ++k) cb[k] = vc0[K * rbd::VC_STRIDE + k];
    rbd::sym6_mv(Ia, cb, Iac);
    double* o = out + (int64_t)tab.depth[K] * rstride * SREC;
#pragma unroll
    for (int k = 0; k < 6; ++k) o[k] = U[k];
    o[6] = dinv;
#pragma unroll
    for (int k = 0; k < 6; ++k) o[7 + k] = Iac[k];
    prev = K;
  }
}

template <class T, bool SP>
struct SpliceCtx {
  using L = QcLayout<T>;
  static constexpr int UQS = 1;
  static constexpr bool V_STEPPED = false;
  static constexpr bool LDS_VEL = false;
  const DevModel* m;
  const double* __restrict__ qc0;
  const double* __restrict__ xg;
  const double* __restrict__ ug;
  const double* __restrict__ spb;
  int rbase, rstride;
  double* uq;
  int i, j;
  unsigned long long ai, aj;
  template <int K> __device__ __forceinline__ const double* er(double*) const {
    const int own = (int)(K == i) | (int)(K == j);
    if constexpr (SP) return qc0 + (K * rbd::QC_STRIDE + own * (L::DELTA + K * L::DW - K * rbd::QC_STRIDE));
    else return qc0 + (K * rbd::QC_STRIDE + own * ((1 + K) * T::N * rbd::QC_STRIDE));
  }
  template <int K> __device__ __forceinline__ const double* ud() const {
    constexpr int DK = depth_of<T>(K);
    if constexpr (desc_mask<T>(K) == 0) return qc0 + (K * rbd::QC_STRIDE + 12);
    else {
      const int si = (int)((ai >> K) & 1), sj = (int)((aj >> K) & 1);
      const int cfg = (si & (sj ^ 1)) * (1 + i) + (sj & (si ^ 1)) * (1 + j);
      const double* p = SP ? qc0 + ((K * rbd::QC_STRIDE + 12) + (si ^ sj) * (L::PATH0 - L::DW + DK * L::UD - (K * rbd::QC_STRIDE + 12)) + cfg * L::DW)
                           : qc0 + ((cfg * T::N + K) * rbd::QC_STRIDE + 12);
      if constexpr (!spine_joint<T>(K)) return p;
      else {
        const double* q = spb + (rbase + DK * rstride) * SREC;
        return (si & sj) ? q : p;
      }
    }
  }
  template <int K> __device__ __forceinline__ const double* er_down(double*) const {
    const int64_t own = (K - i) * (K - j) == 0 ? (SP ? (int64_t)(L::DELTA + K * L::DW - K * rbd::QC_STRIDE) : (int64_t)(1 + K) * T::N * rbd::QC_STRIDE) : 0;
    return qc0 + K * rbd::QC_STRIDE + own;
  }
  template <int K> __device__ __forceinline__ const double* ud_down() const {
    constexpr int DK = depth_of<T>(K);
    if constexpr (desc_mask<T>(K) == 0) return qc0 + (K * rbd::QC_STRIDE + 12);
    else {
      const bool si = (ai >> K) & 1, sj = (aj >> K) & 1;
      const int cfg = sj ? 1 + j : (si ? 1 + i : 0);
      const double* p = SP ? qc0 + (cfg ? (int64_t)(cfg - 1) * L::DW + (L::PATH0 + DK * L::UD) : (int64_t)(K * rbd::QC_STRIDE + 12))
                           : qc0 + (int64_t)cfg * (T::N * rbd::QC_STRIDE) + (K * rbd::QC_STRIDE + 12);
      if constexpr (!spine_joint<T>(K)) return p;
      else {
        const double* q = spb + ((int64_t)rbase + (int64_t)DK * rstride) * SREC;
        return ((ai & aj) >> K) & 1 ? q : p;
      }
    }
  }
  template <int K> __device__ __forceinline__ void ia_cb(const double* ud, const double* cb, double* Iac) const {
    if constexpr (!spine_joint<T>(K)) rbd::sym6_mv(ud + 7, cb, Iac);
    else {
      const int on = (int)(((ai & aj) >> K) & 1);
      const double* pIa = on ? qc0 + (K * rbd::QC_STRIDE + 19) : ud + 7;
      const double w1 = (double)on, w0 = (double)(on ^ 1);
      double t[6];
#pragma unroll
      for (int k = 0; k < 6; ++k) t[k] = ud[7 + k];
      rbd::sym6_mv(pIa, cb, Iac);
#pragma unroll
      for (int k = 0; k < 6; ++k) Iac[k] = w1 * t[k] + w0 * Iac[k];
    }
  }
};
template <class T, bool SP>
__global__ __launch_bounds__(LBS, 2) void lin_static_cfg_pair_kernel(LinParams p, const double* __restrict__ spine, int64_t bt0, int nb) {
  constexpr int nv = T::N, n = 2 * nv;
  constexpr int TRI = nv * (nv - 1) / 2, GU = (TRI + LBS - 1) / LBS, NREC = spine_records<T>();
  int btl, g;
  if (!xcd_slot<GU>(nb, btl, g)) return;
  const int64_t bt = bt0 + btl;
  const int lane = threadIdx.x;
  const int64_t Tn = p.d.T;
  const int b = (int)(bt / Tn);
  const int64_t t = bt % Tn;
  const int slot = g * LBS + lane;
  const bool valid = slot < TRI;
  const int sc = valid ? slot : 0;
  const SpineTab<T>& tab = g_spine_tab<T>;
  __shared__ OutStage<nv> S;
  SpliceCtx<T, SP> c;
  c.i = tab.pi[sc]; c.j = tab.pj[sc];
  c.ai = tab.anc[c.i];
  c.aj = tab.anc[c.j];
  c.rbase = tab.rbase[sc]; c.rstride = tab.rstride[sc];
  c.m = p.model;
  c.qc0 = p.qcache + bt * p.qc_bt;
  c.xg = p.x + ((int64_t)b * (Tn + 1) + t) * n;
  c.ug = p.u + ((int64_t)b * Tn + t) * nv;
  c.spb = spine + (int64_t)btl * NREC * SREC;
  c.uq = &S.qdd[lane * (nv + 1)];
  VelState<T> s;
  chains_up_all<T>(c, s, std::make_integer_sequence<int, nv>{});
  vel_down_all<T>(c, s, std::make_integer_sequence<int, nv>{});
  __builtin_amdgcn_sched_barrier(0);
  offdiag_emit<nv, LBS>(emit_params(), S, valid, c.i, c.j, bt, c.xg, c.m->dt);
}

template <int NV, bool DIAG>
__device__ __forceinline__ void first_output(const double* q , int lane, int d0, double* __restrict__ out,
                                             int64_t ostride, const double* __restrict__ fcol, const double* __restrict__ f0,
                                             const double* __restrict__ xg, double dt, double eps, bool skip_top = false, bool pack = false) {
  constexpr int n = 2 * NV, TOT = NV * n;
  const double eps2 = eps * eps;
  for (int e = lane; e < TOT; e += LBS) {
    const int c = e / n, k = e - c * n;
    const int d = d0 + c;
    if (DIAG && skip_top && k < NV && !(d < n && d % NV == k)) continue;
    double xk = xg[k];
    if (k == d) xk = xk + eps;
    double fv;
    if (k < NV) {
      double xv = xg[NV + k];
      if (NV + k == d) xv = xv + eps;
      const double vo = dt * xv;
      fv = xk + vo;
    } else {
      fv = xk + q[c * (NV + 1) + (k - NV)] * dt;
    }
    if constexpr (DIAG) {
      double df = fv - f0[k];
      df -= eps * fcol[e];
      df *= 2;
      out[rec_row<NV>(pack, k, d < n ? d % NV : -1) + c * ostride] = df / eps2;
    } else {
      out[e] = (fv - f0[k]) / eps;
    }
  }
}

template <class T, int LEVEL, bool DIAG>
__global__ __launch_bounds__(LBS) void lin_static_first_kernel(LinParams p, const DevModel* __restrict__ model, const double* __restrict__ qcache,
                                                               const double* __restrict__ xs, const double* __restrict__ us,
                                                               double* __restrict__ ws, int64_t bt0) {
  constexpr int nv = T::N, n = 2 * nv;
  const int64_t bt = bt0 + blockIdx.x;
  const int lane = threadIdx.x;
  const int64_t Tn = p.d.T;
  const int b = (int)(bt / Tn);
  const int64_t t = bt % Tn;
  const bool valid = lane < nv;
  const double eps = DIAG ? sqrt(sqrt(DBL_EPSILON)) : sqrt(DBL_EPSILON);
  const double* __restrict__ qc0 = qcache + bt * p.qc_bt;
  const double* __restrict__ xg = xs + ((int64_t)b * (Tn + 1) + t) * n;
  const double* __restrict__ ug = us + ((int64_t)b * Tn + t) * nv;
  __shared__ double s_q[(nv + 1) * (nv + 1)];
  double* uq = s_q + (valid ? lane : nv) * (nv + 1);
  if constexpr (LEVEL == 3) {
    const double* __restrict__ vc = p.vcache + (bt * p.nvcfg) * (int64_t)nv * rbd::VC_STRIDE;
    TauState<T> s;
    auto tau = [&](int k) { double v = ug[k]; if (k == lane) v = v + eps; return v; };
    tau_up_all<T, rbd::QC_STRIDE>(*model, qc0, vc, tau, s, std::make_integer_sequence<int, nv>{});
    tau_down_all<T, rbd::QC_STRIDE>(*model, qc0, vc, s, std::make_integer_sequence<int, nv>{});
#pragma unroll
    for (int k = 0; k < nv; ++k) uq[k] = s.uu[k];
  } else if constexpr (LEVEL == 2) {
    VelCtx<1> c;
    c.m = model; c.qc = qc0; c.qp = qc0; c.xg = xg; c.ug = ug; c.uq = uq;
    c.i = nv + lane; c.j = -1; c.eps = eps;
    VelState<T> s;
    chains_up_all<T>(c, s, std::make_integer_sequence<int, nv>{});
    vel_down_all<T>(c, s, std::make_integer_sequence<int, nv>{});
  } else {
    constexpr int MAXCH = max_chain<T>();
    __shared__ double s_vel[MAXCH * 6 * LBS];
    __shared__ double s_own[12 * LBS];
    if constexpr (!DIAG) {
      double E[9], r[3];
      const int jn = valid ? lane : 0;
      rbd::joint_placement(*model, jn, xg[jn] + eps, E, r);
#pragma unroll
      for (int e = 0; e < 9; ++e) s_own[lane * 12 + e] = E[e];
#pragma unroll
      for (int e = 0; e < 3; ++e) s_own[lane * 12 + 9 + e] = r[e];
    }
    CfgCtx<T> c;
    c.m = model; c.qc0 = qc0; c.xg = xg; c.ug = ug;
    c.W = ws + (int64_t)blockIdx.x * (nv * WS_PER_JOINT * LBS) + lane;
    c.lvel = s_vel + lane;
    c.i = valid ? lane : 0; c.j = -1;
    c.own = DIAG ? nullptr : s_own + lane * 12;
    CfgState<T> s;
    chains_up_all<T>(c, s, std::make_integer_sequence<int, nv>{});
#pragma unroll
    for (int e = 0; e < WS_PER_JOINT; ++e) s.w[0][e] = c.W[e * LBS];
    CfgDownOut<nv + 1> o{uq};
    cfg_down_all<T>(c, s, o, std::make_integer_sequence<int, nv>{});
  }
  __builtin_amdgcn_sched_barrier(0);
  const kernarg_t kp = kernarg_params();
  __syncthreads();
  if constexpr (!DIAG) {
    if (double* ao = kp->accel_out) {
      ao += bt * (3 * nv + 1) * nv;
      double* al = ao + (LEVEL - 1) * nv * nv;
      for (int e = lane; e < nv * nv; e += LBS) { const int c = e / nv; al[e] = s_q[c * (nv + 1) + (e - c * nv)]; }
      if (LEVEL == 2 && lane < nv) ao[3 * nv * nv + lane] = s_q[nv * (nv + 1) + lane];
      return;
    }
  }
  double* fcol = LEVEL == 3 ? kp->fu + bt * n * nv : kp->fx + bt * n * n + (LEVEL == 2 ? nv * n : 0);
  double* out = fcol;
  int64_t ostride = n;
  if constexpr (DIAG) {
    const int64_t cs = kp->pack ? nv + 2 : n;
    if (LEVEL == 3) { out = kp->fuu + bt * n * nv * nv; ostride = cs + (int64_t)n * nv; }
    else { ostride = cs + (int64_t)n * n; out = kp->fxx + bt * n * n * n + (LEVEL == 2 ? nv * ostride : 0); }
  }
  first_output<nv, DIAG>(s_q, lane, LEVEL == 1 ? 0 : (LEVEL == 2 ? nv : n), out, ostride, fcol, kp->f_val + bt * n, xg, model->dt, eps, kp->skip_top != 0,
                         DIAG && kp->pack != 0);
}

template <class T, int K>
__device__ __forceinline__ void placement_static(const DevModel& m, double q, double* P) {
  const double* Rp = m.Rp[K];
  const double* a = m.axis[K];
  double* E = P;
  double* r = P + 9;
  if constexpr (!T::prismatic[K]) {
    double sn, cs;
    sincos(q, &sn, &cs);
    const double Kx[9] = {0, -a[2], a[1], a[2], 0, -a[0], -a[1], a[0], 0};
    double K2[9], RJ[9], Rc[9];
    rbd::mm3(Kx, Kx, K2);
    const double omc = 1.0 - cs;
#pragma unroll
    for (int k = 0; k < 9; ++k) RJ[k] = sn * Kx[k] + omc * K2[k];
    RJ[0] += 1.0; RJ[4] += 1.0; RJ[8] += 1.0;
    rbd::mm3(Rp, RJ, Rc);
#pragma unroll
    for (int k = 0; k < 3; ++k)
#pragma unroll
      for (int l = 0; l < 3; ++l) E[3 * k + l] = Rc[3 * l + k];
    r[0] = m.pp[K][0]; r[1] = m.pp[K][1]; r[2] = m.pp[K][2];
  } else {
    const double dd[3] = {a[0] * q, a[1] * q, a[2] * q};
    double Rd[3];
    rbd::mv3(Rp, dd, Rd);
#pragma unroll
    for (int k = 0; k < 3; ++k)
#pragma unroll
      for (int l = 0; l < 3; ++l) E[3 * k + l] = Rp[3 * l + k];
    r[0] = m.pp[K][0] + Rd[0]; r[1] = m.pp[K][1] + Rd[1]; r[2] = m.pp[K][2] + Rd[2];
  }
}

template <class T, bool SP_>
struct QvCtx {
  static constexpr bool SP = SP_;
  static constexpr bool V_STEPPED = false;
  static constexpr bool LDS_VEL = true;
  const DevModel* __restrict__ m;
  const double* __restrict__ xg;
  double* qc;
  double* qown;
  double* qpath;
  unsigned long long anc;
  double* __restrict__ vc;
  double* lvel;
  int jn;
  double eps;
  template <int K> __device__ __forceinline__ const double* er(double* P) const {
    double q = xg[K];
    if (K == jn) q = q + eps;
    placement_static<T, K>(*m, q, P);
    return P;
  }
};
template <class T>
struct QvState {
  double vel[T::N][6];
  double accI[T::N][21];
};
template <class T, int K, int F, bool SP>
__device__ __forceinline__ void chain_up(const QvCtx<T, SP>& c, QvState<T>& s) {
  constexpr int o = T::prismatic[K] ? 3 : 0;
  const double* a = c.m->axis[K];
  double Pb[12], IA[21], U[6], Ia[21], vel[6], dinv;
  const double* P = c.template er<K>(Pb);
  chain_vel_load<T, K, F>(c, s.vel, vel);
  if constexpr (has_child<T>(K)) {
#pragma unroll
    for (int k = 0; k < 21; ++k) IA[k] = s.accI[K][k];
  } else {
#pragma unroll
    for (int k = 0; k < 21; ++k) IA[k] = c.m->I6[K][k];
  }
  step_U_dinv<o>(IA, a, U, dinv);
  step_Ia(IA, U, dinv, Ia);
  constexpr int par = T::parent[K];
  if constexpr (par >= 0) {
    if constexpr (first_contrib<T>(K)) {
#pragma unroll
      for (int k = 0; k < 21; ++k) s.accI[par][k] = c.m->I6[par][k];
    }
    rbd::add_xtix(P, P + 9, Ia, s.accI[par]);
  }
  double vJ[6], vrec[18];
  step_joint_motion<o>(a, lane_v<T::N>(c, K), vJ);
  step_vpart(c.m->I6[K], Ia, vel, vJ, vrec);
  double* qo_er = c.qc + K * rbd::QC_STRIDE;
  double* qo_ud = qo_er + 12;
  if constexpr (SP) {
    constexpr int DK = depth_of<T>(K);
    qo_er = K == c.jn ? c.qown : qo_er;
    if constexpr (has_child<T>(K)) qo_ud = ((c.anc >> K) & 1ull) ? c.qpath + DK * QcLayout<T>::UD : qo_ud;
  }
#pragma unroll
  for (int k = 0; k < 12; ++k) qo_er[k] = P[k];
#pragma unroll
  for (int k = 0; k < 6; ++k) qo_ud[k] = U[k];
  qo_ud[6] = dinv;
#pragma unroll
  for (int k = 0; k < 21; ++k) qo_ud[7 + k] = Ia[k];
  double* vo = c.vc + K * rbd::VC_STRIDE;
#pragma unroll
  for (int k = 0; k < 18; ++k) vo[k] = vrec[k];
  __builtin_amdgcn_sched_barrier(0);
  if constexpr (K > F) chain_up<T, K - 1, F>(c, s);
}

template <class T, bool SP>
__global__ __launch_bounds__(LBS, 2) void lin_static_qvcache_kernel(LinParams p, const DevModel* __restrict__ model, const double* __restrict__ xs,
                                                                 double* __restrict__ qcache, double* __restrict__ vcache) {
  constexpr int nv = T::N, n = 2 * nv, MAXCH = max_chain<T>();
  const int lane = threadIdx.x;
  const int64_t Tn = p.d.T;
  const int64_t e = (int64_t)blockIdx.x * LBS + lane;
  const int64_t bt = e / p.ncfg;
  const int cfgi = (int)(e - bt * p.ncfg);
  const int b = (int)(bt / Tn);
  const int64_t t = bt % Tn;
  __shared__ double s_vel[MAXCH * 6 * LBS];
  if (bt >= p.d.batch * Tn) return;
  QvCtx<T, SP> c;
  c.m = model;
  c.xg = xs + ((int64_t)b * (Tn + 1) + t) * n;
  c.qc = qcache + bt * p.qc_bt + (SP ? 0 : cfgi * (nv * rbd::QC_STRIDE));
  {
    const int g = cfgi > 0 ? cfgi - 1 : 0;
    c.qown = c.qc + (QcLayout<T>::DELTA + g * QcLayout<T>::DW);
    c.qpath = c.qown + QcLayout<T>::ER;
    c.anc = g_anc_tab<T>.anc[g];
  }
  c.vc = vcache + (bt * p.nvcfg + (cfgi == 0 ? 0 : nv + cfgi)) * (int64_t)nv * rbd::VC_STRIDE;
  c.lvel = s_vel + lane;
  c.jn = cfgi - 1;
  c.eps = sqrt(sqrt(DBL_EPSILON));
  QvState<T> s;
  chains_up_all<T>(c, s, std::make_integer_sequence<int, nv>{});
}

template <class T, int K>
__device__ __forceinline__ void vc_joint(const DevModel& m, const double* __restrict__ qc, const double* __restrict__ xg, int iv, double eps,
                                         double (&vel)[T::N][6], double* __restrict__ vc) {
  constexpr int o = T::prismatic[K] ? 3 : 0;
  const double* E = qc + K * rbd::QC_STRIDE;
  const double* r = E + 9;
  const double* Ia = E + 19;
  const double* a = m.axis[K];
  double vK = xg[T::N + K];
  if (K == iv) vK = vK + eps;
  double vJ[6], vrec[18];
  step_joint_motion<o>(a, vK, vJ);
  step_link_vel<(T::parent[K] < 0)>(E, r, vel[T::parent[K] >= 0 ? T::parent[K] : 0], vJ, vel[K]);
  step_vpart(m.I6[K], Ia, vel[K], vJ, vrec);
  double* vo = vc + K * rbd::VC_STRIDE;
#pragma unroll
  for (int k = 0; k < 18; ++k) vo[k] = vrec[k];
  __builtin_amdgcn_sched_barrier(0);
}
template <class T, int... Ks>
__device__ __forceinline__ void vc_all(const DevModel& m, const double* __restrict__ qc, const double* __restrict__ xg, int iv, double eps,
                                       double (&vel)[T::N][6], double* __restrict__ vc, std::integer_sequence<int, Ks...>) {
  (vc_joint<T, Ks>(m, qc, xg, iv, eps, vel, vc), ...);
}
template <class T>
__global__ __launch_bounds__(LBS) void lin_static_vcache_kernel(LinParams p, const DevModel* __restrict__ model, const double* __restrict__ xs,
                                                                const double* __restrict__ qcache, double* __restrict__ vcache) {
  constexpr int nv = T::N, n = 2 * nv;
  const int64_t bt = blockIdx.x;
  const int lane = threadIdx.x;
  const int64_t Tn = p.d.T;
  const int b = (int)(bt / Tn);
  const int64_t t = bt % Tn;
  if (lane >= nv) return;
  const double* __restrict__ qc = qcache + bt * p.qc_bt;
  const double* __restrict__ xg = xs + ((int64_t)b * (Tn + 1) + t) * n;
  double* __restrict__ vc = vcache + (bt * (2 * nv + 1) + 1 + lane) * (int64_t)nv * rbd::VC_STRIDE;
  double vel[nv][6];
  vc_all<T>(*model, qc, xg, lane, sqrt(sqrt(DBL_EPSILON)), vel, vc, std::make_integer_sequence<int, nv>{});
}

}

int lin_static_supported(const DevModel& m) {
  if (m.ff) return 0;
  if (topo_matches<TopoTalos38>(m)) return 1;
  if (topo_matches<TopoChain6>(m)) return 2;
#define DDP_TOPO_MATCH(ID, TOPO) if (topo_matches<TOPO>(m)) return (ID) - 1;
  DDP_TOPO_EXTRA(DDP_TOPO_MATCH)
#undef DDP_TOPO_MATCH
  return 0;
}

int64_t lin_static_qc_per_bt(int topo) {
  if (topo == 1) return QcLayout<TopoTalos38>::WORDS;
  if (topo == 2) return QcLayout<TopoChain6>::WORDS;
#define DDP_TOPO_QC(ID, TOPO) if (topo == (ID) - 1) return QcLayout<TOPO>::WORDS;
  DDP_TOPO_EXTRA(DDP_TOPO_QC)
#undef DDP_TOPO_QC
  return 0;
}

int64_t lin_static_ws_per_bt(const DevModel& m) {
  const int64_t nv = m.nv, TRI = nv * (nv - 1) / 2, GU = (TRI + LBS - 1) / LBS;
  int64_t rec = 0;
  for (int i = 0; i < nv; ++i)
    for (int j = i + 1; j < nv; ++j) {
      const auto anc = [&](int a, int x) { for (int k = m.parent[x]; k >= 0; k = m.parent[k]) if (k == a) return true; return false; };
      int a = m.parent[i];
      while (a >= 0 && !anc(a, j)) a = m.parent[a];
      for (; a >= 0; a = m.parent[a]) ++rec;
    }
  const int64_t sweep = GU * nv * WS_PER_JOINT * LBS, splice = rec * SREC;
  return sweep > splice ? sweep : splice;
}

template <class T>
static void launch_qvcache(const LinParams& p, int64_t BT, hipStream_t s) {
  const dim3 grid((unsigned)((BT * p.ncfg + LBS - 1) / LBS));
  if (p.qc_sparse) hipLaunchKernelGGL((lin_static_qvcache_kernel<T, true>), grid, dim3(LBS), 0, s, p, p.model, p.x, p.qcache, p.vcache);
  else hipLaunchKernelGGL((lin_static_qvcache_kernel<T, false>), grid, dim3(LBS), 0, s, p, p.model, p.x, p.qcache, p.vcache);
}
template <class T>
static void launch_tau_rows(const LinParams& p, int64_t BT, hipStream_t s) {
  const dim3 grid((unsigned)(BT * 2 * T::N));
  if (p.qc_sparse) hipLaunchKernelGGL((lin_static_tau_kernel<T, true, false, true>), grid, dim3(LBS), 0, s, p);
  else hipLaunchKernelGGL((lin_static_tau_kernel<T, true>), grid, dim3(LBS), 0, s, p);
}
template <class T>
static void launch_vel_rows(const LinParams& p, int64_t BT, hipStream_t s) {
  const dim3 grid((unsigned)(BT * T::N));
  if (p.qc_sparse) hipLaunchKernelGGL((lin_static_vel_kernel<T, true, true>), grid, dim3(LBS), 0, s, p);
  else hipLaunchKernelGGL((lin_static_vel_kernel<T, true>), grid, dim3(LBS), 0, s, p);
}

template <class T>
static void launch_first_columns(ddp_hip_ctx* ctx, const LinParams& p, bool with_u) {
  const int64_t BT = ctx->d.batch * ctx->d.T;
  constexpr int nv = T::N, TRI = nv * (nv - 1) / 2, GU = (TRI + LBS - 1) / LBS;
  const int64_t per = ctx->lin_qws_bt * GU;
  for (int64_t bt0 = 0; bt0 < BT; bt0 += per) {
    const int64_t nb = BT - bt0 < per ? BT - bt0 : per;
    hipLaunchKernelGGL((lin_static_first_kernel<T, 1, false>), dim3((unsigned)nb), dim3(LBS), 0, ctx->stream, p, p.model, p.qcache, p.x, p.u, ctx->lin_qws, bt0);
  }
  hipLaunchKernelGGL((lin_static_first_kernel<T, 2, false>), dim3((unsigned)BT), dim3(LBS), 0, ctx->stream, p, p.model, p.qcache, p.x, p.u, ctx->lin_qws, (int64_t)0);
  if (with_u) hipLaunchKernelGGL((lin_static_first_kernel<T, 3, false>), dim3((unsigned)BT), dim3(LBS), 0, ctx->stream, p, p.model, p.qcache, p.x, p.u, ctx->lin_qws, (int64_t)0);
}

template <class T>
static int launch_cfg_slices(ddp_hip_ctx* ctx, const LinParams& p, hipStream_t s, hipEvent_t rows_done) {
  const int64_t BT = ctx->d.batch * ctx->d.T;
  constexpr int nv = T::N, TRI = nv * (nv - 1) / 2, GU = (TRI + LBS - 1) / LBS;
  constexpr int64_t NREC = spine_records<T>(), SWEEP = (int64_t)GU * nv * WS_PER_JOINT * LBS;
  constexpr int64_t WS_BT = SWEEP > NREC * SREC ? SWEEP : NREC * SREC;
  const int64_t per = NREC > 0 ? ctx->lin_qws_bt * WS_BT / (NREC * SREC) : BT;
  for (int64_t bt0 = 0; bt0 < BT; bt0 += per) {
    const int nb = (int)(BT - bt0 < per ? BT - bt0 : per);
    const dim3 grid((unsigned)((nb + 7) / 8 * 8 * GU));
    if (p.qc_sparse) hipLaunchKernelGGL((lin_static_spine_kernel<T, true>), grid, dim3(LBS), 0, s, p.model, p.qcache, p.qc_bt, p.vcache, ctx->lin_qws, bt0, nb);
    else hipLaunchKernelGGL((lin_static_spine_kernel<T, false>), grid, dim3(LBS), 0, s, p.model, p.qcache, p.qc_bt, p.vcache, ctx->lin_qws, bt0, nb);
    if (rows_done) { HIP_TRY(hipStreamWaitEvent(s, rows_done, 0)); rows_done = nullptr; }
    if (p.qc_sparse) hipLaunchKernelGGL((lin_static_cfg_pair_kernel<T, true>), grid, dim3(LBS), 0, s, p, ctx->lin_qws, bt0, nb);
    else hipLaunchKernelGGL((lin_static_cfg_pair_kernel<T, false>), grid, dim3(LBS), 0, s, p, ctx->lin_qws, bt0, nb);
  }
  return DDP_HIP_OK;
}

template <class T>
static int launch_second_order(ddp_hip_ctx* ctx, const LinParams& p) {
  const int64_t BT = ctx->d.batch * ctx->d.T;
  constexpr int nv = T::N, TRI = nv * (nv - 1) / 2, GU = (TRI + LBS - 1) / LBS;
  const bool fork_cfg = (ctx->plan.forks & LIN_FORK_CFG) != 0, spine_ahead = fork_cfg && (ctx->plan.forks & LIN_FORK_SPINE);
  hipStream_t s0 = ctx->stream;
  if (spine_ahead) HIP_TRY(lin_fork(ctx));
  hipLaunchKernelGGL((lin_static_first_kernel<T, 3, true>), dim3((unsigned)BT), dim3(LBS), 0, s0, p, p.model, p.qcache, p.x, p.u, ctx->lin_qws, (int64_t)0);
  launch_tau_rows<T>(p, BT, s0);
  if (fork_cfg) {
    if (spine_ahead) HIP_TRY(hipEventRecord(ctx->lin_ev_rows, s0));
    else HIP_TRY(lin_fork(ctx));
    const int rc_ = launch_cfg_slices<T>(ctx, p, ctx->lin_stream2, spine_ahead ? ctx->lin_ev_rows : nullptr);
    if (rc_ != DDP_HIP_OK) return rc_;
  }
  if (p.pack) hipLaunchKernelGGL((lin_static_tau_kernel<T, false, true>), dim3((unsigned)(BT * GU)), dim3(LBS), 0, s0, p);
  else hipLaunchKernelGGL((lin_static_tau_kernel<T, false, false>), dim3((unsigned)(BT * GU)), dim3(LBS), 0, s0, p);
  launch_vel_rows<T>(p, BT, s0);
  hipLaunchKernelGGL((lin_static_vel_kernel<T, false>), dim3((unsigned)(BT * GU)), dim3(LBS), 0, s0, p);
  if (!fork_cfg) { const int rc_ = launch_cfg_slices<T>(ctx, p, s0, nullptr); if (rc_ != DDP_HIP_OK) return rc_; }
  return DDP_HIP_OK;
}

template <class T>
static int lin_static_launch_t(ddp_hip_ctx* ctx, const LinParams& p, StaticLevel level) {
  const int64_t BT = ctx->d.batch * ctx->d.T;
  constexpr int nv = T::N, TRI = nv * (nv - 1) / 2, GU = (TRI + LBS - 1) / LBS;
  if (level == StaticLevel::Torque) {
    launch_tau_rows<T>(p, BT, ctx->stream);
    if (p.pack) hipLaunchKernelGGL((lin_static_tau_kernel<T, false, true>), dim3((unsigned)(BT * GU)), dim3(LBS), 0, ctx->stream, p);
    else hipLaunchKernelGGL((lin_static_tau_kernel<T, false, false>), dim3((unsigned)(BT * GU)), dim3(LBS), 0, ctx->stream, p);
  } else if (level == StaticLevel::Caches) {
    launch_qvcache<T>(p, BT, ctx->stream);
    if (p.nvcfg > 1) hipLaunchKernelGGL((lin_static_vcache_kernel<T>), dim3((unsigned)BT), dim3(LBS), 0, ctx->stream, p, p.model, p.x, p.qcache, p.vcache);
  } else if (level == StaticLevel::AccelXU || level == StaticLevel::AccelX) {
    if (!p.accel_out) return DDP_HIP_E_ARG;
    launch_qvcache<T>(p, BT, ctx->stream);
    launch_first_columns<T>(ctx, p, level == StaticLevel::AccelXU);
  } else if (level == StaticLevel::FirstOrder) {
    launch_first_columns<T>(ctx, p, true);
  } else if (level == StaticLevel::SecondOrder) {
    { const int rc_ = launch_second_order<T>(ctx, p); if (rc_ != DDP_HIP_OK) return rc_; }
  } else if (level == StaticLevel::UDiagonal) {
    hipLaunchKernelGGL((lin_static_first_kernel<T, 3, true>), dim3((unsigned)BT), dim3(LBS), 0, ctx->stream, p, p.model, p.qcache, p.x, p.u, ctx->lin_qws, (int64_t)0);
  } else if (level == StaticLevel::Configuration && !ctx->sw.cfg_full_aba) {
    { const int rc_ = launch_cfg_slices<T>(ctx, p, ctx->stream, nullptr); if (rc_ != DDP_HIP_OK) return rc_; }
  } else if (level == StaticLevel::Configuration) {
    const int64_t per = ctx->lin_qws_bt;
    hipStream_t s0 = ctx->stream, s1 = ctx->lin_stream2;
    int k = 0;
    for (int64_t bt0 = 0; bt0 < BT; bt0 += per, ++k) {
      const int64_t nb = BT - bt0 < per ? BT - bt0 : per;
      const int w = k & 1;
      double* ws = w ? ctx->lin_qws2 : ctx->lin_qws;
      if (k >= 2) HIP_TRY(hipStreamWaitEvent(s0, ctx->lin_ev_dn[w], 0));
      hipLaunchKernelGGL((lin_static_cfg_up_kernel<T>), dim3((unsigned)(nb * GU)), dim3(LBS), 0, s0, p, p.model, p.qcache, p.x, p.u, ws, bt0);
      HIP_TRY(hipEventRecord(ctx->lin_ev_up[w], s0));
      HIP_TRY(hipStreamWaitEvent(s1, ctx->lin_ev_up[w], 0));
      hipLaunchKernelGGL((lin_static_cfg_down_kernel<T>), dim3((unsigned)(nb * GU)), dim3(LBS), 0, s1, p, p.model, p.qcache, p.x, p.u, ws, bt0);
      HIP_TRY(hipEventRecord(ctx->lin_ev_dn[w], s1));
    }
    if (k >= 1) HIP_TRY(hipStreamWaitEvent(s0, ctx->lin_ev_dn[0], 0));
    if (k >= 2) HIP_TRY(hipStreamWaitEvent(s0, ctx->lin_ev_dn[1], 0));
  } else if (level == StaticLevel::Velocity) {
    launch_vel_rows<T>(p, BT, ctx->stream);
    hipLaunchKernelGGL((lin_static_vel_kernel<T, false>), dim3((unsigned)(BT * GU)), dim3(LBS), 0, ctx->stream, p);
  }
  HIP_TRY(hipGetLastError());
  return DDP_HIP_OK;
}

int lin_static_launch(ddp_hip_ctx* ctx, const LinParams& p, StaticLevel level) {
  if (ctx->plan.topo == 1) return lin_static_launch_t<TopoTalos38>(ctx, p, level);
  if (ctx->plan.topo == 2) return lin_static_launch_t<TopoChain6>(ctx, p, level);
#define DDP_TOPO_LAUNCH(ID, TOPO) if (ctx->plan.topo == (ID) - 1) return lin_static_launch_t<TOPO>(ctx, p, level);
  DDP_TOPO_EXTRA(DDP_TOPO_LAUNCH)
#undef DDP_TOPO_LAUNCH
  return DDP_HIP_E_UNSUPPORTED;
}
```

Before: 807.0.

## Store velocity cache as base plus sparse per-joint deltas

Adds a sparse layout for the velocity cache, mirroring the existing sparse configuration cache. It stores a base block plus, for each perturbed joint, only the records on its ancestor path and subtree, instead of a full nv-record block for each of the 2*nv+1 perturbations. The qv-cache, v-cache, tau-row and spine kernels compute word offsets through a compile-time table. This shrinks workspace and memory traffic in exchange for extra index arithmetic and more complex addressing. The dense layout stays available behind an environment switch.

```diff
diff --git a/ddp_pinocchio_amd/csrc/internal.h b/ddp_pinocchio_amd/csrc/internal.h
--- a/ddp_pinocchio_amd/csrc/internal.h
+++ b/ddp_pinocchio_amd/csrc/internal.h
@@ -59,6 +59,7 @@
   bool no_static = false;
   bool no_qcache = false;
   bool qcache_dense = false;
+  bool vcache_dense = false;
   bool cfg_full_aba = false;
   bool ana_own_aba = false;
   bool ana_split = false;
@@ -126,6 +127,7 @@
   bool m1_fused = false;
   int32_t ncfg = 0, nvcfg = 0;
   bool qc_sparse = false;
+  bool vc_sparse = false;
   bool has_tensors = false;
   bool skip_top = false;
   bool skip_qv_mirror = false;
diff --git a/ddp_pinocchio_amd/csrc/lin.hip b/ddp_pinocchio_amd/csrc/lin.hip
--- a/ddp_pinocchio_amd/csrc/lin.hip
+++ b/ddp_pinocchio_amd/csrc/lin.hip
@@ -1427,6 +1427,11 @@
   return pl.qc_sparse ? lin_static_qc_per_bt(pl.topo) : (int64_t)pl.ncfg * ctx->d.nv * rbd::QC_STRIDE;
 }
 
+int64_t lin_vc_per_bt(const ddp_hip_ctx* ctx) {
+  const LinPlan& pl = ctx->plan;
+  return pl.vc_sparse ? lin_static_vc_per_bt(pl.topo) : (int64_t)pl.nvcfg * ctx->d.nv * rbd::VC_STRIDE;
+}
+
 LinParams make_params(ddp_hip_ctx* ctx) {
   LinParams p{};
   p.d = ctx->d;
@@ -1454,6 +1459,8 @@
   p.qc_sparse = pl.qc_sparse ? 1 : 0;
   p.qc_bt = lin_qc_per_bt(ctx);
   p.vcache = p.qcache ? p.qcache + ctx->d.batch * ctx->d.T * p.qc_bt : nullptr;
+  p.vc_sparse = pl.vc_sparse ? 1 : 0;
+  p.vc_bt = lin_vc_per_bt(ctx);
   p.xref = S(DDP_HIP_SEQ_COST_XREF); p.wx = S(DDP_HIP_SEQ_COST_WX); p.uref = S(DDP_HIP_SEQ_COST_UREF); p.wu = S(DDP_HIP_SEQ_COST_WU);
   return p;
 }
@@ -1685,7 +1692,7 @@
   const LinPlan& pl = ctx->plan;
   if (pl.refuse) return pl.refuse;
   if (pl.ws_lin)
-    HIP_TRY(hipMalloc(&ctx->lin_ws, sizeof(double) * (size_t)(d.batch * d.T * (lin_qc_per_bt(ctx) + (int64_t)pl.nvcfg * d.nv * rbd::VC_STRIDE))));
+    HIP_TRY(hipMalloc(&ctx->lin_ws, sizeof(double) * (size_t)(d.batch * d.T * (lin_qc_per_bt(ctx) + lin_vc_per_bt(ctx)))));
   if (pl.ws_qws) {
     const int64_t BT = d.batch * d.T;
     int64_t slice = (pl.forks & LIN_FORK_SPINE) ? 3200 : 1024;
diff --git a/ddp_pinocchio_amd/csrc/lin_common.h b/ddp_pinocchio_amd/csrc/lin_common.h
--- a/ddp_pinocchio_amd/csrc/lin_common.h
+++ b/ddp_pinocchio_amd/csrc/lin_common.h
@@ -14,6 +14,8 @@
   int32_t has_tensors;
   double *eq_xk, *eq_fxk, *eq_c;
   double* vcache;
+  int64_t vc_bt;
+  int32_t vc_sparse;
   double* qcache;
   int64_t qc_bt;
   int32_t qc_sparse;
@@ -42,6 +44,7 @@
 int lin_static_launch(ddp_hip_ctx* ctx, const LinParams& p, StaticLevel level);
 int64_t lin_static_ws_per_bt(const DevModel& m);
 int64_t lin_static_qc_per_bt(int topo);
+int64_t lin_static_vc_per_bt(int topo);
 
 int lin_analytic_setup(ddp_hip_ctx* ctx);
 void lin_analytic_teardown(ddp_hip_ctx* ctx);
diff --git a/ddp_pinocchio_amd/csrc/lin_plan.cpp b/ddp_pinocchio_amd/csrc/lin_plan.cpp
--- a/ddp_pinocchio_amd/csrc/lin_plan.cpp
+++ b/ddp_pinocchio_amd/csrc/lin_plan.cpp
@@ -15,6 +15,7 @@
   sw.no_static = on("DDP_HIP_NO_STATIC");
   sw.no_qcache = on("DDP_HIP_NO_QCACHE");
   sw.qcache_dense = on("DDP_HIP_QCACHE_DENSE");
+  sw.vcache_dense = on("DDP_HIP_VCACHE_DENSE");
   sw.cfg_full_aba = on("DDP_HIP_CFG_FULL_ABA");
   sw.ana_own_aba = on("DDP_HIP_ANA_OWN_ABA");
   sw.ana_split = on("DDP_HIP_ANA_SPLIT");
@@ -68,6 +69,7 @@
   else pl.second = LinSecond::Mode2Plain;
   pl.ws_qws2 = pl.second == LinSecond::Mode2Static && sw.cfg_full_aba;
   pl.qc_sparse = pl.second == LinSecond::Mode2Static && !sw.qcache_dense && !sw.cfg_full_aba;
+  pl.vc_sparse = pl.qc_sparse && !sw.vcache_dense;
   pl.skip_top = pl.topo && mode == 2 && tensors && !sw.fxx_full;
   pl.skip_qv_mirror = pl.skip_top && sweep_sym_ok;
   pl.pack = pl.skip_qv_mirror && pl.second == LinSecond::Mode2Static && !sw.k3_no_half && !sw.k3_no_pack;
@@ -105,13 +107,14 @@
 #include <stdio.h>
 
 int main(int argc, char** argv) {
-  if (argc > 1 && (argv[1][0] == 's' || argv[1][0] == 'c')) {
+  if (argc > 1 && (argv[1][0] == 's' || argv[1][0] == 'c' || argv[1][0] == 'v')) {
     DevModel m{};
     m.kind = DDP_HIP_MODEL_TREE; m.nv = 38; m.nj = 38; m.nq = 38; m.first_order_fd = 1; m.fd_mode = 2; m.max_level_width = 4;
     Dims d{};
     d.T = 3; d.batch = 2; d.nv = 38; d.n = 76; d.m = 38; d.nx = 76;
     const LinPlan p = lin_plan_decide(m, d, 0u, read_switches(), 1, true);
     if (argv[1][0] == 'c') { printf("qc_sparse %d ncfg %d nvcfg %d\n", (int)p.qc_sparse, p.ncfg, p.nvcfg); return 0; }
+    if (argv[1][0] == 'v') { printf("vc_sparse %d qc_sparse %d nvcfg %d\n", (int)p.vc_sparse, (int)p.qc_sparse, p.nvcfg); return 0; }
     printf("forks %u topo %d\n", p.forks, p.topo);
     return 0;
   }
diff --git a/ddp_pinocchio_amd/csrc/lin_static.hip b/ddp_pinocchio_amd/csrc/lin_static.hip
--- a/ddp_pinocchio_amd/csrc/lin_static.hip
+++ b/ddp_pinocchio_amd/csrc/lin_static.hip
@@ -84,6 +84,43 @@
   const int base = K * rbd::QC_STRIDE + e, own = L::DELTA + g * L::DW + e, path = L::PATH0 + g * L::DW + d * L::UD + (e - L::ER);
   const int w_own = (int)(e < L::ER) & (int)(K == g), w_path = (int)(e >= L::ER) & (int)((anc >> K) & 1ull);
   return base + w_own * (own - base) + w_path * (path - base);
+}
+
+template <class T>
+struct VcTab { int qoff[T::N], voff[T::N], sub[T::N]; int words; };
+template <class T>
+constexpr VcTab<T> make_vc_tab() {
+  constexpr int N = T::N, R = rbd::VC_STRIDE;
+  VcTab<T> t{};
+  int depth[N] = {};
+  for (int k = 0; k < N; ++k)
+    for (int a = T::parent[k]; a >= 0; a = T::parent[a]) { ++depth[k]; ++t.sub[a]; }
+  for (int k = 0; k < N; ++k) ++t.sub[k];
+  int off = 2 * N * R;
+  for (int g = 0; g < N; ++g) { t.qoff[g] = off; off += (depth[g] + t.sub[g]) * R; }
+  for (int g = 0; g < N; ++g) { t.voff[g] = off; off += t.sub[g] * R; }
+  t.words = off;
+  return t;
+}
+template <class T>
+struct VcLayout {
+  static constexpr int N = T::N, R = rbd::VC_STRIDE;
+  static constexpr int VB = N * R;
+  static constexpr int WORDS = make_vc_tab<T>().words;
+};
+template <class T> __device__ const VcTab<T> g_vc_tab = make_vc_tab<T>();
+template <class T>
+__device__ __forceinline__ int vc_word(int kind, int g, unsigned long long anc, int K, int e) {
+  using L = VcLayout<T>;
+  const VcTab<T>& tab = g_vc_tab<T>;
+  const int gi = g < 0 ? 0 : g;
+  const int nsub = g < 0 ? 0 : tab.sub[gi];
+  const int off = kind ? tab.voff[gi] : tab.qoff[gi];
+  const unsigned long long a = kind ? 0ull : anc;
+  const int dg = __popcll(a), d = __popcll(a & ((1ull << K) - 1ull));
+  const int base = kind * L::VB + K * L::R + e, below = off + (dg + K - g) * L::R + e, path = off + d * L::R + e;
+  const int w_below = (int)(K >= g) & (int)(K < g + nsub), w_path = (int)((a >> K) & 1ull);
+  return base + w_below * (below - base) + w_path * (path - base);
 }
 template <class T>
 struct TauState {
@@ -217,8 +254,9 @@
       rv[c] = vc[K0 * rbd::VC_STRIDE + idx];
     }
   }
-  template <class T>
-  __device__ __forceinline__ void load_sparse(const double* __restrict__ qc0, int g, unsigned long long anc, const double* __restrict__ vc, int lane) {
+  template <class T, bool VSP>
+  __device__ __forceinline__ void load_sparse(const double* __restrict__ qc0, int g, unsigned long long anc, const double* __restrict__ vc,
+                                              int vkind, int vg, unsigned long long vanc, int lane) {
 #pragma unroll
     for (int c = 0; c < CP; ++c) {
       int idx = c * LBS + lane;
@@ -230,7 +268,12 @@
     for (int c = 0; c < CV; ++c) {
       int idx = c * LBS + lane;
       idx = idx < NVW ? idx : NVW - 1;
-      rv[c] = vc[K0 * rbd::VC_STRIDE + idx];
+      if constexpr (VSP) {
+        const int K = K0 + idx / rbd::VC_STRIDE, e = idx % rbd::VC_STRIDE;
+        rv[c] = vc[vc_word<T>(vkind, vg, vanc, K, e)];
+      } else {
+        rv[c] = vc[K0 * rbd::VC_STRIDE + idx];
+      }
     }
   }
   __device__ __forceinline__ void park(double* sp, double* sv, int lane) const {
@@ -489,7 +532,7 @@
   return po;
 }
 
-template <class T, bool ROWS, bool PACK = false, bool SP = false>
+template <class T, bool ROWS, bool PACK = false, bool SP = false, bool VSP = false>
 __global__ __launch_bounds__(LBS, ROWS ? 1 : 3) void lin_static_tau_kernel(LinParams p) {
   constexpr int nv = T::N, n = 2 * nv;
   constexpr int TRI = nv * (nv - 1) / 2, GU = (TRI + LBS - 1) / LBS, G = ROWS ? 2 * nv : GU;
@@ -513,12 +556,14 @@
   const double eps = sqrt(sqrt(DBL_EPSILON));
   static_assert(ROWS || !SP, "the pairs read the base block alone");
   const double* __restrict__ qc = p.qcache + bt * p.qc_bt + (SP ? 0 : cfg * (nv * rbd::QC_STRIDE));
-  const double* __restrict__ vc = p.vcache + (bt * (2 * nv + 1) + vcfg) * (int64_t)nv * rbd::VC_STRIDE;
+  static_assert(SP || !VSP, "the base + deltas v-cache comes with the base + deltas q-cache");
+  const double* __restrict__ vc = p.vcache + bt * p.vc_bt + (VSP ? 0 : vcfg * (nv * rbd::VC_STRIDE));
   const double* __restrict__ xg = p.x + ((int64_t)b * (Tn + 1) + t) * n;
   const double* __restrict__ ug = p.u + ((int64_t)b * Tn + t) * nv;
   const int iu = i - n, ju = j - n;
   const int gq = cfg - 1;
   [[maybe_unused]] const unsigned long long ganc = SP && cfg > 0 ? g_anc_tab<T>.anc[gq] : 0ull;
+  [[maybe_unused]] const int vkind = g < nv ? 0 : 1, vg = g < nv ? g : g - nv;
   __shared__ union TauLds { double P[nv * PS + nv * rbd::VC_STRIDE]; RowStage<nv> S; OutStage<nv, LBS / 2> O; } s_lds;
   double* s_P = s_lds.P;
   double* s_V = s_P + nv * PS;
@@ -526,7 +571,7 @@
   StageRegs<nv, 0, (KH > 0) ? KH : 1> lower;
   {
     StageRegs<nv, KH, nv> upper;
-    if constexpr (SP) { upper.template load_sparse<T>(qc, gq, ganc, vc, lane); lower.template load_sparse<T>(qc, gq, ganc, vc, lane); }
+    if constexpr (SP) { upper.template load_sparse<T, VSP>(qc, gq, ganc, vc, vkind, vg, ganc, lane); lower.template load_sparse<T, VSP>(qc, gq, ganc, vc, vkind, vg, ganc, lane); }
     else { upper.load(qc, vc, lane); lower.load(qc, vc, lane); }
     upper.park(s_P, s_V, lane);
     rbd::coop_sync<true>();
@@ -1145,7 +1190,7 @@
 
 template <class T, bool SP>
 __global__ __launch_bounds__(LBS) void lin_static_spine_kernel(const DevModel* __restrict__ model, const double* __restrict__ qcache, int64_t qc_bt,
-                                                               const double* __restrict__ vcache, double* __restrict__ spine, int64_t bt0, int nb) {
+                                                               const double* __restrict__ vcache, int64_t vc_bt, double* __restrict__ spine, int64_t bt0, int nb) {
   constexpr int nv = T::N, TRI = nv * (nv - 1) / 2, GU = (TRI + LBS - 1) / LBS, NREC = spine_records<T>();
   int btl, g;
   if (!xcd_slot<GU>(nb, btl, g)) return;
@@ -1157,7 +1202,7 @@
   const int rstride = tab.rstride[slot];
   [[maybe_unused]] const unsigned long long anc_i = tab.anc[i], anc_j = tab.anc[j];
   const double* __restrict__ qc0 = qcache + (bt0 + btl) * qc_bt;
-  const double* __restrict__ vc0 = vcache + ((bt0 + btl) * (2 * nv + 1)) * (int64_t)nv * rbd::VC_STRIDE;
+  const double* __restrict__ vc0 = vcache + (bt0 + btl) * vc_bt;
   double* __restrict__ out = spine + ((int64_t)btl * NREC + tab.rbase[slot]) * SREC;
   double Ia[21];
 #pragma unroll
@@ -1372,7 +1417,7 @@
   __shared__ double s_q[(nv + 1) * (nv + 1)];
   double* uq = s_q + (valid ? lane : nv) * (nv + 1);
   if constexpr (LEVEL == 3) {
-    const double* __restrict__ vc = p.vcache + (bt * p.nvcfg) * (int64_t)nv * rbd::VC_STRIDE;
+    const double* __restrict__ vc = p.vcache + bt * p.vc_bt;
     TauState<T> s;
     auto tau = [&](int k) { double v = ug[k]; if (k == lane) v = v + eps; return v; };
     tau_up_all<T, rbd::QC_STRIDE>(*model, qc0, vc, tau, s, std::make_integer_sequence<int, nv>{});
@@ -1470,9 +1515,9 @@
   }
 }
 
-template <class T, bool SP_>
+template <class T, bool SP_, bool VSP_>
 struct QvCtx {
-  static constexpr bool SP = SP_;
+  static constexpr bool SP = SP_, VSP = VSP_;
   static constexpr bool V_STEPPED = false;
   static constexpr bool LDS_VEL = true;
   const DevModel* __restrict__ m;
@@ -1482,6 +1527,9 @@
   double* qpath;
   unsigned long long anc;
   double* __restrict__ vc;
+  int vpath;
+  int vsub;
+  int sub_end;
   double* lvel;
   int jn;
   double eps;
@@ -1497,8 +1545,8 @@
   double vel[T::N][6];
   double accI[T::N][21];
 };
-template <class T, int K, int F, bool SP>
-__device__ __forceinline__ void chain_up(const QvCtx<T, SP>& c, QvState<T>& s) {
+template <class T, int K, int F, bool SP, bool VSP>
+__device__ __forceinline__ void chain_up(const QvCtx<T, SP, VSP>& c, QvState<T>& s) {
   constexpr int o = T::prismatic[K] ? 3 : 0;
   const double* a = c.m->axis[K];
   double Pb[12], IA[21], U[6], Ia[21], vel[6], dinv;
@@ -1538,14 +1586,20 @@
   qo_ud[6] = dinv;
 #pragma unroll
   for (int k = 0; k < 21; ++k) qo_ud[7 + k] = Ia[k];
-  double* vo = c.vc + K * rbd::VC_STRIDE;
+  int voff = K * rbd::VC_STRIDE;
+  if constexpr (VSP) {
+    constexpr int DK = depth_of<T>(K);
+    voff = (K >= c.jn) & (K < c.sub_end) ? c.vsub + K * rbd::VC_STRIDE : voff;
+    if constexpr (has_child<T>(K)) voff = ((c.anc >> K) & 1ull) ? c.vpath + DK * rbd::VC_STRIDE : voff;
+  }
+  double* vo = c.vc + voff;
 #pragma unroll
   for (int k = 0; k < 18; ++k) vo[k] = vrec[k];
   __builtin_amdgcn_sched_barrier(0);
   if constexpr (K > F) chain_up<T, K - 1, F>(c, s);
 }
 
-template <class T, bool SP>
+template <class T, bool SP, bool VSP = false>
 __global__ __launch_bounds__(LBS, 2) void lin_static_qvcache_kernel(LinParams p, const DevModel* __restrict__ model, const double* __restrict__ xs,
                                                                  double* __restrict__ qcache, double* __restrict__ vcache) {
   constexpr int nv = T::N, n = 2 * nv, MAXCH = max_chain<T>();
@@ -1558,7 +1612,8 @@
   const int64_t t = bt % Tn;
   __shared__ double s_vel[MAXCH * 6 * LBS];
   if (bt >= p.d.batch * Tn) return;
-  QvCtx<T, SP> c;
+  static_assert(SP || !VSP, "the base + deltas v-cache comes with the base + deltas q-cache");
+  QvCtx<T, SP, VSP> c;
   c.m = model;
   c.xg = xs + ((int64_t)b * (Tn + 1) + t) * n;
   c.qc = qcache + bt * p.qc_bt + (SP ? 0 : cfgi * (nv * rbd::QC_STRIDE));
@@ -1567,8 +1622,11 @@
     c.qown = c.qc + (QcLayout<T>::DELTA + g * QcLayout<T>::DW);
     c.qpath = c.qown + QcLayout<T>::ER;
     c.anc = g_anc_tab<T>.anc[g];
-  }
-  c.vc = vcache + (bt * p.nvcfg + (cfgi == 0 ? 0 : nv + cfgi)) * (int64_t)nv * rbd::VC_STRIDE;
+    c.vc = vcache + bt * p.vc_bt + (VSP || cfgi == 0 ? 0 : (nv + cfgi) * (nv * rbd::VC_STRIDE));
+    c.vpath = g_vc_tab<T>.qoff[g];
+    c.vsub = c.vpath + (__popcll(c.anc) - g) * rbd::VC_STRIDE;
+    c.sub_end = cfgi > 0 ? g + g_vc_tab<T>.sub[g] : 0;
+  }
   c.lvel = s_vel + lane;
   c.jn = cfgi - 1;
   c.eps = sqrt(sqrt(DBL_EPSILON));
@@ -1576,9 +1634,9 @@
   chains_up_all<T>(c, s, std::make_integer_sequence<int, nv>{});
 }
 
-template <class T, int K>
+template <class T, int K, bool VSP>
 __device__ __forceinline__ void vc_joint(const DevModel& m, const double* __restrict__ qc, const double* __restrict__ xg, int iv, double eps,
-                                         double (&vel)[T::N][6], double* __restrict__ vc) {
+                                         double (&vel)[T::N][6], double* __restrict__ vc, int vown, int sub_end) {
   constexpr int o = T::prismatic[K] ? 3 : 0;
   const double* E = qc + K * rbd::QC_STRIDE;
   const double* r = E + 9;
@@ -1590,17 +1648,19 @@
   step_joint_motion<o>(a, vK, vJ);
   step_link_vel<(T::parent[K] < 0)>(E, r, vel[T::parent[K] >= 0 ? T::parent[K] : 0], vJ, vel[K]);
   step_vpart(m.I6[K], Ia, vel[K], vJ, vrec);
-  double* vo = vc + K * rbd::VC_STRIDE;
+  int voff = K * rbd::VC_STRIDE;
+  if constexpr (VSP) voff = (K >= iv) & (K < sub_end) ? vown + K * rbd::VC_STRIDE : voff;
+  double* vo = vc + voff;
 #pragma unroll
   for (int k = 0; k < 18; ++k) vo[k] = vrec[k];
   __builtin_amdgcn_sched_barrier(0);
 }
-template <class T, int... Ks>
+template <class T, bool VSP, int... Ks>
 __device__ __forceinline__ void vc_all(const DevModel& m, const double* __restrict__ qc, const double* __restrict__ xg, int iv, double eps,
-                                       double (&vel)[T::N][6], double* __restrict__ vc, std::integer_sequence<int, Ks...>) {
-  (vc_joint<T, Ks>(m, qc, xg, iv, eps, vel, vc), ...);
-}
-template <class T>
+                                       double (&vel)[T::N][6], double* __restrict__ vc, int vown, int sub_end, std::integer_sequence<int, Ks...>) {
+  (vc_joint<T, Ks, VSP>(m, qc, xg, iv, eps, vel, vc, vown, sub_end), ...);
+}
+template <class T, bool VSP>
 __global__ __launch_bounds__(LBS) void lin_static_vcache_kernel(LinParams p, const DevModel* __restrict__ model, const double* __restrict__ xs,
                                                                 const double* __restrict__ qcache, double* __restrict__ vcache) {
   constexpr int nv = T::N, n = 2 * nv;
@@ -1609,12 +1669,16 @@
   const int64_t Tn = p.d.T;
   const int b = (int)(bt / Tn);
   const int64_t t = bt % Tn;
-  if (lane >= nv) return;
+  if (lane >= nv + (VSP ? 1 : 0)) return;
   const double* __restrict__ qc = qcache + bt * p.qc_bt;
   const double* __restrict__ xg = xs + ((int64_t)b * (Tn + 1) + t) * n;
-  double* __restrict__ vc = vcache + (bt * (2 * nv + 1) + 1 + lane) * (int64_t)nv * rbd::VC_STRIDE;
+  double* vc0 = vcache + bt * p.vc_bt;
+  double* vc = vc0 + (VSP ? VcLayout<T>::VB : (1 + lane) * (nv * rbd::VC_STRIDE));
+  const int g = lane < nv ? lane : 0;
+  const int vown = g_vc_tab<T>.voff[g] - g * rbd::VC_STRIDE - VcLayout<T>::VB;
+  const int sub_end = lane < nv ? g + g_vc_tab<T>.sub[g] : 0;
   double vel[nv][6];
-  vc_all<T>(*model, qc, xg, lane, sqrt(sqrt(DBL_EPSILON)), vel, vc, std::make_integer_sequence<int, nv>{});
+  vc_all<T, VSP>(*model, qc, xg, lane, sqrt(sqrt(DBL_EPSILON)), vel, vc, vown, sub_end, std::make_integer_sequence<int, nv>{});
 }
 
 }
@@ -1635,6 +1699,15 @@
 #define DDP_TOPO_QC(ID, TOPO) if (topo == (ID) - 1) return QcLayout<TOPO>::WORDS;
   DDP_TOPO_EXTRA(DDP_TOPO_QC)
 #undef DDP_TOPO_QC
+  return 0;
+}
+
+int64_t lin_static_vc_per_bt(int topo) {
+  if (topo == 1) return VcLayout<TopoTalos38>::WORDS;
+  if (topo == 2) return VcLayout<TopoChain6>::WORDS;
+#define DDP_TOPO_VC(ID, TOPO) if (topo == (ID) - 1) return VcLayout<TOPO>::WORDS;
+  DDP_TOPO_EXTRA(DDP_TOPO_VC)
+#undef DDP_TOPO_VC
   return 0;
 }
 
@@ -1655,13 +1728,15 @@
 template <class T>
 static void launch_qvcache(const LinParams& p, int64_t BT, hipStream_t s) {
   const dim3 grid((unsigned)((BT * p.ncfg + LBS - 1) / LBS));
-  if (p.qc_sparse) hipLaunchKernelGGL((lin_static_qvcache_kernel<T, true>), grid, dim3(LBS), 0, s, p, p.model, p.x, p.qcache, p.vcache);
+  if (p.vc_sparse) hipLaunchKernelGGL((lin_static_qvcache_kernel<T, true, true>), grid, dim3(LBS), 0, s, p, p.model, p.x, p.qcache, p.vcache);
+  else if (p.qc_sparse) hipLaunchKernelGGL((lin_static_qvcache_kernel<T, true>), grid, dim3(LBS), 0, s, p, p.model, p.x, p.qcache, p.vcache);
   else hipLaunchKernelGGL((lin_static_qvcache_kernel<T, false>), grid, dim3(LBS), 0, s, p, p.model, p.x, p.qcache, p.vcache);
 }
 template <class T>
 static void launch_tau_rows(const LinParams& p, int64_t BT, hipStream_t s) {
   const dim3 grid((unsigned)(BT * 2 * T::N));
-  if (p.qc_sparse) hipLaunchKernelGGL((lin_static_tau_kernel<T, true, false, true>), grid, dim3(LBS), 0, s, p);
+  if (p.vc_sparse) hipLaunchKernelGGL((lin_static_tau_kernel<T, true, false, true, true>), grid, dim3(LBS), 0, s, p);
+  else if (p.qc_sparse) hipLaunchKernelGGL((lin_static_tau_kernel<T, true, false, true>), grid, dim3(LBS), 0, s, p);
   else hipLaunchKernelGGL((lin_static_tau_kernel<T, true>), grid, dim3(LBS), 0, s, p);
 }
 template <class T>
@@ -1694,8 +1769,8 @@
   for (int64_t bt0 = 0; bt0 < BT; bt0 += per) {
     const int nb = (int)(BT - bt0 < per ? BT - bt0 : per);
     const dim3 grid((unsigned)((nb + 7) / 8 * 8 * GU));
-    if (p.qc_sparse) hipLaunchKernelGGL((lin_static_spine_kernel<T, true>), grid, dim3(LBS), 0, s, p.model, p.qcache, p.qc_bt, p.vcache, ctx->lin_qws, bt0, nb);
-    else hipLaunchKernelGGL((lin_static_spine_kernel<T, false>), grid, dim3(LBS), 0, s, p.model, p.qcache, p.qc_bt, p.vcache, ctx->lin_qws, bt0, nb);
+    if (p.qc_sparse) hipLaunchKernelGGL((lin_static_spine_kernel<T, true>), grid, dim3(LBS), 0, s, p.model, p.qcache, p.qc_bt, p.vcache, p.vc_bt, ctx->lin_qws, bt0, nb);
+    else hipLaunchKernelGGL((lin_static_spine_kernel<T, false>), grid, dim3(LBS), 0, s, p.model, p.qcache, p.qc_bt, p.vcache, p.vc_bt, ctx->lin_qws, bt0, nb);
     if (rows_done) { HIP_TRY(hipStreamWaitEvent(s, rows_done, 0)); rows_done = nullptr; }
     if (p.qc_sparse) hipLaunchKernelGGL((lin_static_cfg_pair_kernel<T, true>), grid, dim3(LBS), 0, s, p, ctx->lin_qws, bt0, nb);
     else hipLaunchKernelGGL((lin_static_cfg_pair_kernel<T, false>), grid, dim3(LBS), 0, s, p, ctx->lin_qws, bt0, nb);
@@ -1736,7 +1811,8 @@
     else hipLaunchKernelGGL((lin_static_tau_kernel<T, false, false>), dim3((unsigned)(BT * GU)), dim3(LBS), 0, ctx->stream, p);
   } else if (level == StaticLevel::Caches) {
     launch_qvcache<T>(p, BT, ctx->stream);
-    if (p.nvcfg > 1) hipLaunchKernelGGL((lin_static_vcache_kernel<T>), dim3((unsigned)BT), dim3(LBS), 0, ctx->stream, p, p.model, p.x, p.qcache, p.vcache);
+    if (p.nvcfg > 1 && p.vc_sparse) hipLaunchKernelGGL((lin_static_vcache_kernel<T, true>), dim3((unsigned)BT), dim3(LBS), 0, ctx->stream, p, p.model, p.x, p.qcache, p.vcache);
+    else if (p.nvcfg > 1) hipLaunchKernelGGL((lin_static_vcache_kernel<T, false>), dim3((unsigned)BT), dim3(LBS), 0, ctx->stream, p, p.model, p.x, p.qcache, p.vcache);
   } else if (level == StaticLevel::AccelXU || level == StaticLevel::AccelX) {
     if (!p.accel_out) return DDP_HIP_E_ARG;
     launch_qvcache<T>(p, BT, ctx->stream);
```

Result: faster. 817.3 (median of 6 runs) (+1.3%).
